# lppllppl920/SAGE-SLAM

Measured on AMD Instinct MI355X. Metric: M residuals/sec (+ LM iters/sec), 64-keyframe feature-metric BA @128x160, higher is better.
Workload: dtype f32; 1 GPU; 64-keyframe window, 128x160x16 feature pyramids (L=4), 32-dim depth code, dense sampling N=16128, 186 links = 372 photometric + 372 geometric directed edges; parallelism=single GPU, collective=none, accepted_steps=988

## Files before the change

include/sage_ba.h:

```cpp
#ifndef SAGE_BA_H_
#define SAGE_BA_H_

#include <stddef.h>
#include <stdint.h>

#ifdef __cplusplus
extern "C" {
#endif

#define SAGE_MAX_LEVELS 8
#define SAGE_POSE_FLOATS 12

#define SAGE_OK 0
#define SAGE_E_INVALID (-1)
#define SAGE_E_UNSUPPORTED (-2)
#define SAGE_E_NOT_PSD (-3)
#define SAGE_E_STATE (-4)
#define SAGE_E_NO_OVERLAP (-5)

typedef struct SageCamera
{
  float fx, fy, cx, cy, w, h;
} SageCamera;

// ... 9 lines not shown

const char *sage_version(void);
const char *sage_error_string(int code);

typedef struct SageWorkspace SageWorkspace;
int sage_workspace_create(void *hip_stream, SageWorkspace **out);
void sage_workspace_destroy(SageWorkspace *ws);


int sage_photometric_jac_error_calculate(
    SageWorkspace *ws, float *AtA_dev, float *Atb_dev, float *error_host, float *num_inliers_host,
    const float *R10_dev, const float *t10_dev, const float *R0_dev, const float *t0_dev,
    const float *R1_dev, const float *t1_dev,
    const float *bias0_dev, const float *basis0_dev, const float *code0_dev, const float *mask1_dev,
    const int64_t *loc1d_dev, const float *homo_dev,
    const float *feat0_dev, const float *feat1_dev, const float *grad1_dev,
    float scale0, const SagePyramid *pyr, float eps, const float *weights_host,
    int N, int FS, int CS);

int sage_photometric_error_calculate(
    SageWorkspace *ws, float *error_host, float *num_inliers_host,
    const float *R10_dev, const float *t10_dev,
    const float *bias0_dev, const float *basis0_dev, const float *code0_dev, const float *mask1_dev,
    const int64_t *loc1d_dev, const float *homo_dev,
    const float *feat0_dev, const float *feat1_dev,
    float scale0, const SagePyramid *pyr, float eps, const float *weights_host,
    int N, int FS, int CS);

int sage_tracker_photo_jac_error_calculate(
    SageWorkspace *ws, int dof, float *AtA_dev, float *Atb_dev, float *error_host, float *num_inliers_host,
    const float *R_dev, const float *t_dev, const float *mask1_dev,
    const float *dpts0_dev, const float *homo_dev, const float *feat0s_dev,
    const float *feat1_dev, const float *grad1_dev,
    const SagePyramid *pyr, float scale0, float eps, const float *weights_dev, int N, int FS);

int sage_tracker_photo_error_calculate(
    SageWorkspace *ws, float *error_host, float *num_inliers_host,
    const float *R_dev, const float *t_dev, const float *mask1_dev,
    const float *dpts0_dev, const float *homo_dev, const float *feat0s_dev, const float *feat1_dev,
    const SagePyramid *pyr, float eps, const float *weights_dev, int N, int FS);

int sage_geometric_jac_error_calculate(
    SageWorkspace *ws, float *AtA_dev, float *Atb_dev, float *error_host, float *num_inliers_host,
    const float *R10_dev, const float *t10_dev, const float *R0_dev, const float *t0_dev,
    const float *R1_dev, const float *t1_dev,
    const float *bias0_dev, const float *basis0_dev, const float *code0_dev,
    const float *dpt1_dev, const float *dpt_grad1_dev, const float *basis1_dev, const float *mask1_dev,
    const int32_t *loc1d_dev, const float *homo_dev,
    float scale0, float scale1, const SageCamera *cam, float eps, float loss_param, float weight,
    int N, int CS);

int sage_geometric_error_calculate(
    SageWorkspace *ws, float *error_host, float *num_inliers_host,
    const float *R10_dev, const float *t10_dev,
    const float *bias0_dev, const float *basis0_dev, const float *code0_dev,
    const float *dpt1_dev, const float *mask1_dev, const int32_t *loc1d_dev, const float *homo_dev,
    float scale0, const SageCamera *cam, float eps, float loss_param, float weight, int N, int CS);

int sage_depth_and_grad(SageWorkspace *ws, float *dpt_dev, float *dpt_grad_dev,
                        const float *bias_dev, const float *basis_dev, const float *code_dev,
                        float scale, int H, int W, int CS);
int sage_gaussian_pyramid_with_grad(SageWorkspace *ws, float *pyr_dev, float *grad_dev,
                                    const float *feat_dev, const float *mask_dev,
                                    const SagePyramid *pyr, int FS);

int sage_bind_thread_to_device(int device);
int sage_solver_helper_cpus(int *cpus, int n);
int sage_solver_placement_moves(void);
int sage_placement_monitor(int enable);
void sage_shutdown(void);
int sage_host_threads_running(void);

void sage_se3_exp(const float *omega, const float *v, float *R, float *t);
void sage_pose_retract(const float *pose, const float *delta6, float *out);
int sage_nearest_psd(const double *M, int n, double *out);
int sage_nearest_psd_reference(const double *M, int n, double *out);
int sage_factor_block_count(int type, int CS);
int sage_factor_hessian_blocks(int type, int CS, const float *AtA_host, const float *Atb_host, int psd_mode,
                               double *G_out, double *g_out, int32_t *dims_out, int32_t *nkeys_out);
int sage_damped_solve_qr_f32(const float *A, const float *b, int n, float damp, float *x);

int sage_block_solve(const double *packed_host, int K, int nlinks, const int32_t *links, int B, double damp,
                     const double *diag_add, const double *g_add, double *delta);
long long sage_solve_lookahead_count(void);

typedef struct SageLmConfig
{
  int max_num_iters;
  float min_grad_thresh;
  float min_param_inc_thresh;
  float init_damp;
  float min_damp, max_damp;
  float damp_dec_factor;
  float damp_inc_factor;
  float jac_update_err_inc_threshold;
  int max_inner_evals;
  float no_overlap_error;
  int linearize_at_candidate;
} SageLmConfig;
void sage_lm_config_default(SageLmConfig *cfg);

typedef int (*SageTrackLinearizeFn)(void *ctx, const float *pose12, float scale, float *AtA, float *Atb, float *error);
typedef int (*SageTrackErrorFn)(void *ctx, const float *pose12, float scale, float *error);

typedef struct SageLmTraceEntry
{
  float damp, error, candidate_error;
  int accepted, relinearized;
} SageLmTraceEntry;

int sage_track_lm(const SageLmConfig *cfg, int dof, SageTrackLinearizeFn lin, SageTrackErrorFn err, void *ctx,
                  float *pose12, float *scale, float *final_error, int *iters,
                  SageLmTraceEntry *trace, int trace_cap, int *trace_len);

typedef struct SageTrackProblem
{
  SageWorkspace *ws;
  int32_t use_photo;
  const float *mask1_dev, *dpts0_dev, *homo_dev, *feat0s_dev, *feat1_dev, *grad1_dev;
  const float *weights_dev;
  SagePyramid pyr;
  float eps;
  int32_t N, FS;
  int32_t use_keypoints, NK;
  const float *kp_dpts0_dev;
  const float *kp_homo0_dev;
  const float *kp_matched_2d_dev;
  const float *kp_matched_dpts1_dev;
  const float *kp_matched_homo1_dev;
  float kp_loss_param;
  float kp_weight;
} SageTrackProblem;
int sage_track_frame(const SageLmConfig *cfg, int dof, const SageTrackProblem *prob,
                     float *pose12, float *scale, float *final_error, int *iters,
                     SageLmTraceEntry *trace, int trace_cap, int *trace_len);

typedef struct SageWindow SageWindow;

typedef struct SageKeyframeView
{
  const float *feat_pyr;
  const float *grad_pyr;
  const float *bias;
  const float *basis;
  const int64_t *loc1d;
  const float *homo;
  int32_t N;
} SageKeyframeView;

typedef struct SageWindowConfig
{
  SagePyramid pyr;
  int32_t FS, CS;
  const float *mask_dev;
  float photo_weights[SAGE_MAX_LEVELS];
  float geo_weight, geo_loss_param, eps;
  float code_prior_weight;
  float scale_prior_weight;
  float pose_prior_weight;
  int32_t use_photo, use_geo;
} SageWindowConfig;

int sage_window_create(const SageWindowConfig *cfg, void *hip_stream, SageWindow **out);
void sage_window_destroy(SageWindow *w);
int sage_window_add_keyframe(SageWindow *w, const SageKeyframeView *view, const float *pose12,
                             const float *code, float scale);
// ... 75 lines not shown
                                        const float *matched_2d, const SageCamera *cam, float eps, float loss_param,
                                        float weight, int N);

enum { SAGE_LOSS_FAIR = 0, SAGE_LOSS_L2 = 1, SAGE_LOSS_HUBER = 2, SAGE_LOSS_UNBIASED = 3 };
int sage_match_geometry_jac_error_calculate(SageWorkspace *ws, float *AtA_dev, float *Atb_dev, float *error_host,
                                            const float *R10, const float *t10, const float *R0, const float *t0,
                                            const float *R1, const float *t1, const float *bias0, const float *bias1,
                                            const float *basis0, const float *basis1, const float *code0,
                                            const float *code1, const float *homo0, const float *matched_homo1,
                                            const int32_t *loc1d_0, const int32_t *matched_loc1d_1, float scale0,
                                            float scale1, float loss_param, float weight, int loss, int N, int CS);
int sage_match_geometry_error_calculate(SageWorkspace *ws, float *error_host, const float *R10, const float *t10,
                                        const float *bias0, const float *bias1, const float *basis0, const float *basis1,
                                        const float *code0, const float *code1, const float *homo0,
                                        const float *matched_homo1, const int32_t *loc1d_0,
                                        const int32_t *matched_loc1d_1, float scale0, float scale1, float loss_param,
                                        float weight, int loss, int N, int CS);
int sage_loop_mg_jac_error_calculate(SageWorkspace *ws, float *AtA_dev, float *Atb_dev, float *error_host,
                                     const float *R10, const float *t10, const float *R0, const float *t0,
                                     const float *R1, const float *t1, const float *unscaled_dpts0,
                                     const float *matched_unscaled_dpts1, const float *homo0, const float *matched_homo1,
                                     float scale0, float scale1, float loss_param, float weight, int N);
int sage_loop_mg_error_calculate(SageWorkspace *ws, float *error_host, const float *R10, const float *t10,
                                 const float *unscaled_dpts0, const float *matched_unscaled_dpts1, const float *homo0,
                                 const float *matched_homo1, float scale0, float scale1, float loss_param, float weight,
                                 int N);
int sage_tracker_match_geom_jac_error_calculate(SageWorkspace *ws, float *AtA_dev, float *Atb_dev, float *error_host,
                                                const float *R, const float *t, const float *sampled_dpts0,
                                                const float *matched_dpts1, const float *homo0,
                                                const float *matched_homo1, float scale0, float loss_param,
                                                float weight, int with_scale, int N);
int sage_tracker_match_geom_error_calculate(SageWorkspace *ws, float *error_host, const float *R, const float *t,
                                            const float *sampled_dpts0, const float *matched_dpts1, const float *homo0,
                                            const float *matched_homo1, float loss_param, float weight, int N);

int sage_cycle_match(SageWorkspace *ws, const float *desc0_dev, const float *desc1_dev, const int64_t *kp_loc1d_0,
                     int K, int C, int H, int W, float cyc_thresh, int64_t *raw_matched_loc1d_1,
                     int64_t *cyc_matched_loc1d_0, int32_t *inlier_flags, int *n_inliers_host);

int sage_sort_locations(SageWorkspace *ws, const int64_t *loc1d_dev, const float *homo_dev, int n, int H, int W,
                        int64_t *loc1d_out_dev, float *homo_out_dev, int *sorted_host);
int sage_valid_locations(SageWorkspace *ws, const float *mask_dev, const SageCamera *cam, int64_t *loc1d_dev,
                         float *homo_dev, int *n_valid_host);
int sage_shuffle_indices(int64_t seed, int64_t n, int64_t *idx_host);
int sage_sample_locations(SageWorkspace *ws, const int64_t *valid_loc1d_dev, const float *valid_homo_dev, int n_valid,
                          int64_t seed, int num_samples, int64_t *loc1d_dev, float *homo_dev, int *n_out_host);

typedef int (*SageAllReduceFn)(double *dev_buf, size_t n, void *user);
int sage_window_set_allreduce(SageWindow *w, SageAllReduceFn fn, void *user);

typedef struct SageShardPlan SageShardPlan;
int sage_shard_plan_create(int K, int nlinks, const int32_t *links, int B, int rank, int world, SageShardPlan **out);
void sage_shard_plan_destroy(SageShardPlan *p);
size_t sage_shard_sep_count(const SageShardPlan *p);
int sage_shard_num_separators(const SageShardPlan *p);
int sage_shard_num_interior(const SageShardPlan *p);
int sage_shard_keyframe_owner(const SageShardPlan *p, int kf);
int sage_shard_keyframe_is_local(const SageShardPlan *p, int kf);
int sage_shard_eliminate(SageShardPlan *p, const double *packed_local_host, double damp, const double *diag_add,
                         const double *g_add, double *sep_out);
int sage_shard_solve(SageShardPlan *p, const double *sep_reduced, double *delta);
int sage_shard_plan_create_domains(int K, int nlinks, const int32_t *links, int B, int domain, int ndomains,
                                   SageShardPlan **out);
int sage_block_solve_domains(const double *packed_host, int K, int nlinks, const int32_t *links, int B, double damp,
                             const double *diag_add, const double *g_add, int ndomains, double *delta);

int sage_window_emulate_peers(SageWindow *w, const double *rest_dev, int n_iterates);
#define SAGE_RCCL_ID_BYTES 128
int sage_rccl_unique_id(unsigned char *id128);
int sage_rccl_comm_create(const unsigned char *id128, int rank, int world, void **comm_out);
void sage_rccl_comm_destroy(void *comm);
int sage_rccl_comm_info(void *comm, int *ranks_out, int *rank_out);
int sage_window_use_rccl(SageWindow *w, void *nccl_comm);

typedef struct SageLmState
{
  double damp, error, candidate_error;
  int accepted, iters;
} SageLmState;
int sage_window_lm_step(SageWindow *w, SageLmState *st, const SageLmConfig *cfg);
int sage_window_lm_run(SageWindow *w, SageLmState *st, const SageLmConfig *cfg, int n, double *trace, int *done);
int sage_window_lm_run_timed(SageWindow *w, SageLmState *st, const SageLmConfig *cfg, int n, double *trace, int *done,
                             double *step_seconds);
int sage_window_sync_variables(SageWindow *w);

#ifdef __cplusplus
}
#endif
#endif
```

sage_slam_amd/build.py:

```python
from __future__ import annotations

import os
import subprocess
import sys
from concurrent.futures import ThreadPoolExecutor

HERE = os.path.dirname(os.path.abspath(__file__))
ROOT = os.path.dirname(HERE)
CSRC = os.path.join(HERE, "csrc")
OBJ = os.path.join(HERE, "csrc", "_obj")
LIB = os.path.join(HERE, "libsage_ba.so")
SOURCES = ["photo_kernels.hip", "geo_kernels.hip", "track_kernels.hip", "producers.hip", "keypoint_kernels.hip", "solve_kernels.hip", "operators.hip", "tracker.hip", "window.hip", "window_build.hip", "window_dist.hip", "window_factors.hip",
           "host_math.cpp", "block_solver.cpp", "host_threads.cpp", "shard_solve.cpp"]
HEADERS = ["sage_device.h", "sage_internal.h", "host_math.h", "block_solver.h", "host_threads.h", "runtime_internal.h", "finalize_bodies.h", "keypoint_batch.h", "window_plan.h", os.path.join(ROOT, "include", "sage_ba.h")]
HIPCC = os.environ.get("HIPCC", "/opt/rocm/bin/hipcc")
HOSTCXX = os.environ.get("HOSTCXX", "/opt/rocm/lib/llvm/bin/clang++")
FLAGS = ["--offload-arch=gfx950", "-O3", "-std=c++17", "-fPIC", "-Wall", "-Wno-unused-function",
         "-I" + os.path.join(ROOT, "include"), "-I" + CSRC]


def kernel_source_sha16() -> str:
    import hashlib
    h = hashlib.sha256()
    for f in ("photo_kernels.hip", "geo_kernels.hip", "sage_device.h", "sage_internal.h"):
        with open(os.path.join(CSRC, f), "rb") as fh:
            h.update(fh.read())
    return h.hexdigest()[:16]


def _mtime(p):
    return os.path.getmtime(p) if os.path.exists(p) else 0.0


def _compile(src):
    obj = os.path.join(OBJ, os.path.splitext(src)[0] + ".o")
    deps = [os.path.join(CSRC, src)] + [h if os.path.isabs(h) else os.path.join(CSRC, h) for h in HEADERS]
    if _mtime(obj) >= max(_mtime(d) for d in deps):
        return obj, False
    if src.endswith(".hip"):
        cmd = [HIPCC] + FLAGS + ["-x", "hip", "-c", os.path.join(CSRC, src), "-o", obj]
    else:
        cmd = [HOSTCXX, "-O3", "-std=c++17", "-fPIC", "-Wall", "-I" + os.path.join(ROOT, "include"), "-I" + CSRC,
               "-c", os.path.join(CSRC, src), "-o", obj]
    subprocess.check_call(cmd)
    return obj, True


def build(force: bool = False, verbose: bool = False) -> str:
    os.makedirs(OBJ, exist_ok=True)
    if force:
        for f in os.listdir(OBJ):
            os.remove(os.path.join(OBJ, f))
    with ThreadPoolExecutor(max_workers=min(8, len(SOURCES))) as ex:
        res = list(ex.map(_compile, SOURCES))
    objs = [o for o, _ in res]
    if any(ch for _, ch in res) or not os.path.exists(LIB):
        subprocess.check_call([HIPCC, "--offload-arch=gfx950", "-shared", "-fPIC", "-o", LIB] + objs + ["-lpthread"])
        if verbose:
            print("built", LIB)
    return LIB


GLUE_SRC = os.path.join(ROOT, "integration", "compile_check", "prepass_run.cpp")
GLUE_BIN = os.path.join(ROOT, "integration", "compile_check", "_bin", "prepass_run")
REF_THIRDPARTY = "/root/reference/system/thirdparty"


def build_glue_check(verbose: bool = False):
    if not os.path.isdir(REF_THIRDPARTY):
        return GLUE_BIN if os.path.exists(GLUE_BIN) else None
    deps = [GLUE_SRC, os.path.join(ROOT, "integration", "sage_gtsam_prepass.h"), os.path.join(ROOT, "include", "sage_ba.h"),
            os.path.join(ROOT, "integration", "compile_check", "gtsam", "linear", "HessianFactor.h"),
            os.path.join(ROOT, "integration", "compile_check", "gtsam", "nonlinear", "Values.h"), LIB]
    if _mtime(GLUE_BIN) >= max(_mtime(d) for d in deps):
        return GLUE_BIN
    os.makedirs(os.path.dirname(GLUE_BIN), exist_ok=True)
    subprocess.check_call([HOSTCXX, "-std=c++17", "-O1", "-w", "-D__HIP_PLATFORM_AMD__", "-I" + os.path.join(ROOT, "include"),
                           "-I" + os.path.join(ROOT, "integration", "compile_check"), "-I" + REF_THIRDPARTY + "/eigen",
                           "-I" + REF_THIRDPARTY + "/Sophus", "-I/opt/rocm/include", GLUE_SRC, "-o", GLUE_BIN,
                           "-L" + HERE, "-lsage_ba", "-L/opt/rocm/lib", "-lamdhip64",
                           "-Wl,-rpath,$ORIGIN/../../../sage_slam_amd", "-Wl,-rpath,/opt/rocm/lib"])
    if verbose:
        print("built", GLUE_BIN)
    return GLUE_BIN


ADAPTER_BIN = os.path.join(ROOT, "integration", "compile_check", "_bin", "adapter_run")
REF_SYSTEM = "/root/reference/system"


def build_adapter_run(verbose: bool = False):
    if not os.path.isdir(REF_SYSTEM):
        return ADAPTER_BIN if os.path.exists(ADAPTER_BIN) else None
    import torch
    T = os.path.dirname(torch.__file__)
    srcs = [os.path.join(ROOT, "integration", "sage_adapter.cpp"), os.path.join(ROOT, "integration", "sage_adapter_keypoints.cpp"),
            os.path.join(ROOT, "integration", "compile_check", "adapter_run.cpp")]
# ... 31 lines not shown
```

sage_slam_amd/capi.py:

```python
from __future__ import annotations

import ctypes as C
import os
from typing import List, Optional, Sequence

import numpy as np

HERE = os.path.dirname(os.path.abspath(__file__))
LIB_PATH = os.path.join(HERE, "libsage_ba.so")
SAGE_MAX_LEVELS = 8


class SageError(RuntimeError):
    def __init__(self, code: int, where: str):
        self.code = code
        msg = lib().sage_error_string(code).decode() if _lib is not None else "?"
        super().__init__(f"{where}: {msg} (code {code})")


class SageCamera(C.Structure):
    _fields_ = [(n, C.c_float) for n in ("fx", "fy", "cx", "cy", "w", "h")]


class SagePyramid(C.Structure):
    _fields_ = [("levels", C.c_int32), ("P", C.c_int32), ("level_offsets", C.c_int32 * SAGE_MAX_LEVELS),
                ("cam", SageCamera * SAGE_MAX_LEVELS)]


class SageLmConfig(C.Structure):
    _fields_ = [("max_num_iters", C.c_int), ("min_grad_thresh", C.c_float), ("min_param_inc_thresh", C.c_float),
                ("init_damp", C.c_float), ("min_damp", C.c_float), ("max_damp", C.c_float),
                ("damp_dec_factor", C.c_float), ("damp_inc_factor", C.c_float),
                ("jac_update_err_inc_threshold", C.c_float), ("max_inner_evals", C.c_int),
                ("no_overlap_error", C.c_float), ("linearize_at_candidate", C.c_int)]


class SageLmTraceEntry(C.Structure):
    _fields_ = [("damp", C.c_float), ("error", C.c_float), ("candidate_error", C.c_float),
                ("accepted", C.c_int), ("relinearized", C.c_int)]


class SageTrackProblem(C.Structure):
    _fields_ = [("ws", C.c_void_p), ("use_photo", C.c_int32), ("mask1_dev", C.c_void_p), ("dpts0_dev", C.c_void_p),
                ("homo_dev", C.c_void_p), ("feat0s_dev", C.c_void_p), ("feat1_dev", C.c_void_p),
                ("grad1_dev", C.c_void_p), ("weights_dev", C.c_void_p), ("pyr", SagePyramid), ("eps", C.c_float),
                ("N", C.c_int32), ("FS", C.c_int32), ("use_keypoints", C.c_int32), ("NK", C.c_int32),
                ("kp_dpts0_dev", C.c_void_p), ("kp_homo0_dev", C.c_void_p), ("kp_matched_2d_dev", C.c_void_p),
                ("kp_matched_dpts1_dev", C.c_void_p), ("kp_matched_homo1_dev", C.c_void_p),
                ("kp_loss_param", C.c_float), ("kp_weight", C.c_float)]


class SageKeyframeView(C.Structure):
    _fields_ = [("feat_pyr", C.c_void_p), ("grad_pyr", C.c_void_p), ("bias", C.c_void_p), ("basis", C.c_void_p),
                ("loc1d", C.c_void_p), ("homo", C.c_void_p), ("N", C.c_int32)]


class SageWindowConfig(C.Structure):
    _fields_ = [("pyr", SagePyramid), ("FS", C.c_int32), ("CS", C.c_int32), ("mask_dev", C.c_void_p),
                ("photo_weights", C.c_float * SAGE_MAX_LEVELS), ("geo_weight", C.c_float),
                ("geo_loss_param", C.c_float), ("eps", C.c_float), ("code_prior_weight", C.c_float),
                ("scale_prior_weight", C.c_float), ("pose_prior_weight", C.c_float),
                ("use_photo", C.c_int32), ("use_geo", C.c_int32)]


SAGE_KP_REPROJECTION, SAGE_KP_MATCH_GEOMETRY = 0, 1


class SageKeypointTerm(C.Structure):
    _fields_ = [("kind", C.c_int32), ("edge", C.c_int32), ("N", C.c_int32), ("loc1d_0", C.c_void_p), ("homo0", C.c_void_p),
                ("matched_2d", C.c_void_p), ("matched_loc1d_1", C.c_void_p), ("matched_homo1", C.c_void_p),
                ("loss_param", C.c_float), ("weight", C.c_float), ("loss", C.c_int32)]


ALLREDUCE_FN = C.CFUNCTYPE(C.c_int, C.c_void_p, C.c_size_t, C.c_void_p)


class SageLmState(C.Structure):
    _fields_ = [("damp", C.c_double), ("error", C.c_double), ("candidate_error", C.c_double),
                ("accepted", C.c_int), ("iters", C.c_int)]


TRACK_LIN_FN = C.CFUNCTYPE(C.c_int, C.c_void_p, C.POINTER(C.c_float), C.c_float, C.POINTER(C.c_float),
                           C.POINTER(C.c_float), C.POINTER(C.c_float))
TRACK_ERR_FN = C.CFUNCTYPE(C.c_int, C.c_void_p, C.POINTER(C.c_float), C.c_float, C.POINTER(C.c_float))

_lib = None

SYMBOLS = [
    "sage_camera_pyramid", "sage_version", "sage_error_string", "sage_workspace_create", "sage_workspace_destroy",
    "sage_photometric_jac_error_calculate", "sage_photometric_error_calculate",
    "sage_tracker_photo_jac_error_calculate", "sage_tracker_photo_error_calculate",
    "sage_geometric_jac_error_calculate", "sage_geometric_error_calculate", "sage_depth_and_grad",
    "sage_gaussian_pyramid_with_grad", "sage_se3_exp", "sage_pose_retract", "sage_nearest_psd", "sage_nearest_psd_reference", "sage_factor_block_count", "sage_factor_hessian_blocks",
    "sage_damped_solve_qr_f32", "sage_block_solve", "sage_solve_lookahead_count", "sage_lm_config_default", "sage_track_lm", "sage_track_frame",
    "sage_window_create", "sage_window_destroy", "sage_window_add_keyframe", "sage_window_add_link", "sage_window_set_link_geo_loss",
    "sage_window_set_shard", "sage_window_finalize", "sage_window_num_keyframes", "sage_window_num_links",
    "sage_window_block_size", "sage_window_packed_count", "sage_window_packed_dev",
    "sage_window_residuals_per_linearize", "sage_window_bytes_per_linearize", "sage_window_linearize",
    "sage_window_error", "sage_window_tune_runs", "sage_window_set_runs", "sage_window_error_dev", "sage_window_solve", "sage_window_total_error",
    "sage_window_accept", "sage_window_reset", "sage_window_get_keyframe", "sage_window_set_keyframe", "sage_window_get_delta",
    "sage_window_get_edge", "sage_window_add_keypoint_term", "sage_window_num_keypoint_terms", "sage_window_get_keypoint_term", "sage_window_prepass", "sage_window_factor", "sage_window_factor_error", "sage_window_prepare_factors", "sage_factor_psd", "sage_factor_cut_blocks", "sage_window_set_profiling", "sage_window_get_kernel_time", "sage_window_get_phase_time", "sage_window_lm_step", "sage_window_lm_run", "sage_window_lm_run_timed", "sage_window_sync_variables", "sage_window_set_allreduce", "sage_shard_plan_create", "sage_shard_plan_create_domains", "sage_block_solve_domains", "sage_shard_plan_destroy", "sage_shard_sep_count", "sage_shard_num_separators", "sage_shard_num_interior", "sage_shard_keyframe_owner", "sage_shard_keyframe_is_local", "sage_shard_eliminate", "sage_shard_solve", "sage_rccl_unique_id", "sage_rccl_comm_create", "sage_rccl_comm_destroy", "sage_rccl_comm_info", "sage_window_use_rccl", "sage_window_emulate_peers", "sage_sort_locations", "sage_bind_thread_to_device", "sage_solver_helper_cpus", "sage_solver_placement_moves", "sage_placement_monitor", "sage_shutdown", "sage_host_threads_running",
    "sage_valid_locations", "sage_shuffle_indices", "sage_sample_locations",
    "sage_reprojection_jac_error_calculate", "sage_reprojection_error_calculate",
    "sage_tracker_reproj_jac_error_calculate", "sage_tracker_reproj_error_calculate",
    "sage_match_geometry_jac_error_calculate", "sage_match_geometry_error_calculate",
    "sage_loop_mg_jac_error_calculate", "sage_loop_mg_error_calculate",
    "sage_tracker_match_geom_jac_error_calculate", "sage_tracker_match_geom_error_calculate", "sage_cycle_match",
]


def lib():
    global _lib
    if _lib is None:
        LIB_PATH = os.environ.get("SAGE_BA_LIB", globals()["LIB_PATH"])
        if not os.path.exists(LIB_PATH):
            raise ImportError(f"{LIB_PATH} is missing: run `python -m sage_slam_amd.build` "
                              "(the HIP engine has no fallback path)")
        import torch
        L = C.CDLL(LIB_PATH)
        L.sage_version.restype = C.c_char_p
        L.sage_error_string.restype = C.c_char_p
        L.sage_window_packed_count.restype = C.c_size_t
        L.sage_shutdown.restype = None
        L.sage_window_packed_dev.restype = C.c_void_p
        L.sage_window_error_dev.restype = C.c_void_p
        L.sage_window_residuals_per_linearize.restype = C.c_double
        L.sage_window_bytes_per_linearize.restype = C.c_double
        for name in ("sage_window_packed_count", "sage_window_packed_dev", "sage_window_error_dev",
                     "sage_window_residuals_per_linearize", "sage_window_bytes_per_linearize",
                     "sage_window_num_keyframes", "sage_window_num_links", "sage_window_block_size"):
            getattr(L, name).argtypes = [C.c_void_p]
        _lib = L
    return _lib


def _chk(code: int, where: str):
    if code != 0:
        raise SageError(code, where)


def _f32(a) -> np.ndarray:
    return np.ascontiguousarray(a, dtype=np.float32)


def _fp(a: np.ndarray):
    return a.ctypes.data_as(C.POINTER(C.c_float))


def dptr(t) -> C.c_void_p:
    if t is None:
        return C.c_void_p(0)
    assert t.is_contiguous(), "device buffers handed to the C ABI must be contiguous"
    return C.c_void_p(t.data_ptr())


def make_pyramid(cam, levels: int) -> SagePyramid:
    base = SageCamera(*[float(v) for v in (cam.fx, cam.fy, cam.cx, cam.cy, cam.w, cam.h)])
    out = SagePyramid()
    _chk(lib().sage_camera_pyramid(C.byref(base), levels, C.byref(out)), "sage_camera_pyramid")
    return out


def se3_exp(omega, v):
    omega = _f32(omega); v = _f32(v)
    R = np.zeros(9, np.float32); t = np.zeros(3, np.float32)
    lib().sage_se3_exp(_fp(omega), _fp(v), _fp(R), _fp(t))
    return R.reshape(3, 3), t


def pose_retract(pose12, delta6):
    pose12 = _f32(pose12).reshape(12); delta6 = _f32(delta6)
    out = np.zeros(12, np.float32)
    lib().sage_pose_retract(_fp(pose12), _fp(delta6), _fp(out))
    return out


def nearest_psd(M):
    M = np.ascontiguousarray(M, dtype=np.float64)
    out = np.zeros_like(M)
    _chk(lib().sage_nearest_psd(M.ctypes.data_as(C.POINTER(C.c_double)), M.shape[0],
                                out.ctypes.data_as(C.POINTER(C.c_double))), "sage_nearest_psd")
    return out


def nearest_psd_reference(M):
    M = np.ascontiguousarray(M, np.float64)
    out = np.zeros_like(M)
    _chk(lib().sage_nearest_psd_reference(M.ctypes.data_as(C.POINTER(C.c_double)), M.shape[0],
                                          out.ctypes.data_as(C.POINTER(C.c_double))), "sage_nearest_psd_reference")
    return out


def factor_hessian_blocks(type_: int, CS: int, AtA, Atb, psd_mode: int = 1):
    L = lib()
    A = _f32(AtA); b = _f32(Atb)
    n = L.sage_factor_block_count(type_, CS)
    if n < 0:
        raise SageError(n, "sage_factor_block_count")
    G = np.zeros(n, np.float64); g = np.zeros(b.size, np.float64)
    dims = (C.c_int32 * 6)(); nk = C.c_int32()
    _chk(L.sage_factor_hessian_blocks(type_, CS, _fp(A), _fp(b), psd_mode, G.ctypes.data_as(C.POINTER(C.c_double)),
                                      g.ctypes.data_as(C.POINTER(C.c_double)), dims, C.byref(nk)),
         "sage_factor_hessian_blocks")
    dims = [int(dims[i]) for i in range(nk.value)]
    blocks, o = {}, 0
    for i in range(nk.value):
        for j in range(i, nk.value):
            blocks[(i, j)] = G[o:o + dims[i] * dims[j]].reshape(dims[i], dims[j]); o += dims[i] * dims[j]
    offs = np.concatenate([[0], np.cumsum(dims)])
    return blocks, [g[offs[i]:offs[i + 1]] for i in range(nk.value)], dims


def damped_solve_qr_f32(A, b, damp):
    A = _f32(A); b = _f32(b)
    x = np.zeros(b.shape[0], np.float32)
    _chk(lib().sage_damped_solve_qr_f32(_fp(A), _fp(b), b.shape[0], C.c_float(damp), _fp(x)), "sage_damped_solve_qr_f32")
    return x


def block_solve(packed, K, links, B, damp, diag_add=None, g_add=None):
    packed = np.ascontiguousarray(packed, dtype=np.float64)
    lk = np.ascontiguousarray(np.asarray(links, dtype=np.int32).reshape(-1))
    delta = np.zeros(K * B, np.float64)
    dp = lambda a: None if a is None else np.ascontiguousarray(a, np.float64).ctypes.data_as(C.POINTER(C.c_double))
    da = None if diag_add is None else np.ascontiguousarray(diag_add, np.float64)
    ga = None if g_add is None else np.ascontiguousarray(g_add, np.float64)
    _chk(lib().sage_block_solve(packed.ctypes.data_as(C.POINTER(C.c_double)), K, len(lk) // 2, lk.ctypes.data_as(C.POINTER(C.c_int32)), B,
                                C.c_double(damp), dp(da), dp(ga), delta.ctypes.data_as(C.POINTER(C.c_double))),
         "sage_block_solve")
    return delta


def solve_lookahead_count() -> int:
    f = lib().sage_solve_lookahead_count
    f.restype = C.c_longlong
    return int(f())


def block_solve_domains(packed, K, links, B, damp, ndomains, diag_add=None, g_add=None):
    p = np.ascontiguousarray(packed, np.float64)
    lk = np.ascontiguousarray(np.asarray(links, np.int32).reshape(-1))
    out = np.zeros(K * B, np.float64)
    dp = lambda a: None if a is None else np.ascontiguousarray(a, np.float64).ctypes.data_as(C.POINTER(C.c_double))
    da = None if diag_add is None else np.ascontiguousarray(diag_add, np.float64)
    ga = None if g_add is None else np.ascontiguousarray(g_add, np.float64)
    _chk(lib().sage_block_solve_domains(p.ctypes.data_as(C.POINTER(C.c_double)), K, len(links),
                                        lk.ctypes.data_as(C.POINTER(C.c_int32)), B, C.c_double(damp), dp(da), dp(ga),
                                        ndomains, out.ctypes.data_as(C.POINTER(C.c_double))), "sage_block_solve_domains")
    return out


def lm_config_default() -> SageLmConfig:
    cfg = SageLmConfig()
    lib().sage_lm_config_default(C.byref(cfg))
    return cfg


def pack_pose(R, t) -> np.ndarray:
    return np.concatenate([_f32(R).reshape(9), _f32(t).reshape(3)])


def track_lm(cfg: SageLmConfig, dof: int, lin_fn, err_fn, pose12, scale: float, trace_cap: int = 256):
    def _lin(ctx, p, s, AtA, Atb, err):
        A, b, e = lin_fn(np.ctypeslib.as_array(p, (12,)).copy(), float(s))
        A = _f32(A).reshape(-1); b = _f32(b).reshape(-1)
        for i in range(dof * dof):
            AtA[i] = A[i]
        for i in range(dof):
            Atb[i] = b[i]
        err[0] = e
        return 0

    def _err(ctx, p, s, err):
        err[0] = err_fn(np.ctypeslib.as_array(p, (12,)).copy(), float(s))
        return 0

    pose = _f32(pose12).reshape(12).copy()
    sc = C.c_float(scale)
    fe = C.c_float(0); it = C.c_int(0); tl = C.c_int(0)
    trace = (SageLmTraceEntry * trace_cap)()
    cb1, cb2 = TRACK_LIN_FN(_lin), TRACK_ERR_FN(_err)
    _chk(lib().sage_track_lm(C.byref(cfg), dof, cb1, cb2, None, _fp(pose), C.byref(sc), C.byref(fe), C.byref(it),
                             trace, trace_cap, C.byref(tl)), "sage_track_lm")
    tr = [dict(damp=trace[i].damp, error=trace[i].error, candidate_error=trace[i].candidate_error,
               accepted=trace[i].accepted, relinearized=trace[i].relinearized) for i in range(tl.value)]
    return pose, sc.value, fe.value, it.value, tr


def track_frame(cfg: SageLmConfig, dof: int, prob: "SageTrackProblem", pose12, scale: float, trace_cap: int = 256):
    L = lib()
    p = _f32(pose12).copy()
    sc = C.c_float(scale); fe = C.c_float(); it = C.c_int(); tl = C.c_int()
    tr = (SageLmTraceEntry * trace_cap)()
    rc = L.sage_track_frame(C.byref(cfg), dof, C.byref(prob), _fp(p), C.byref(sc), C.byref(fe), C.byref(it), tr,
                            trace_cap, C.byref(tl))
    trace = [dict(damp=tr[i].damp, error=tr[i].error, candidate_error=tr[i].candidate_error,
                  accepted=tr[i].accepted, relinearized=tr[i].relinearized) for i in range(tl.value)]
    return rc, p, sc.value, fe.value, it.value, trace


class Workspace:

    def __init__(self, stream=None):
        self.h = C.c_void_p()
        sp = C.c_void_p(stream.cuda_stream) if stream is not None else C.c_void_p(0)
        _chk(lib().sage_workspace_create(sp, C.byref(self.h)), "sage_workspace_create")

    def close(self):
        if self.h:
            lib().sage_workspace_destroy(self.h)
            self.h = C.c_void_p()

    def __del__(self):
# ... 257 lines not shown
    def tune_runs(self):
        tpb, rule = C.c_int(0), C.c_int(0)
        ms_rule, ms_best = C.c_float(0), C.c_float(0)
        _chk(lib().sage_window_tune_runs(self.h, C.byref(tpb), C.byref(rule), C.byref(ms_rule), C.byref(ms_best)),
             "sage_window_tune_runs")
        return dict(tpb=tpb.value, tpb_rule=rule.value, ms_rule=ms_rule.value, ms_best=ms_best.value)

    def set_runs(self, tpb):
        _chk(lib().sage_window_set_runs(self.h, int(tpb)), "sage_window_set_runs")

    def solve(self, damp, want_norm=True):
        if not want_norm:
            _chk(lib().sage_window_solve(self.h, C.c_double(damp), None), "sage_window_solve")
            return None
        sn = C.c_double()
        _chk(lib().sage_window_solve(self.h, C.c_double(damp), C.byref(sn)), "sage_window_solve")
        return sn.value

    def total_error(self, from_linearize: bool):
        e = C.c_double()
        _chk(lib().sage_window_total_error(self.h, int(from_linearize), C.byref(e)), "sage_window_total_error")
        return e.value

    def accept(self):
        _chk(lib().sage_window_accept(self.h), "sage_window_accept")

    def reset(self):
        _chk(lib().sage_window_reset(self.h), "sage_window_reset")

    def set_allreduce(self, dist_module, group=None):
        tensors = {}
        for t in (self.packed_tensor(), self.error_tensor()):
            tensors[(t.data_ptr(), t.numel())] = t

        def hook(ptr, n, _user):
            try:
                t = tensors.get((ptr, n))
                if t is None:
                    t = tensors[(ptr, n)] = _tensor_from_ptr(ptr, n)
                dist_module.all_reduce(t, group=group)
                return 0
            except Exception:
                import traceback
                traceback.print_exc()
                return 1

        self._allreduce_cb = ALLREDUCE_FN(hook)
        _chk(lib().sage_window_set_allreduce(self.h, self._allreduce_cb, None), "sage_window_set_allreduce")

    def sync_variables(self):
        _chk(lib().sage_window_sync_variables(self.h), "sage_window_sync_variables")

    def use_rccl(self, comm):
        _chk(lib().sage_window_use_rccl(self.h, C.c_void_p(comm)), "sage_window_use_rccl")

    def emulate_peers(self, rest):
        if rest is None:
            self._emu_rest = None
            _chk(lib().sage_window_emulate_peers(self.h, None, 0), "sage_window_emulate_peers")
            return
        assert rest.is_cuda and rest.dim() == 2 and rest.shape[1] == self.packed_count and rest.is_contiguous()
        self._emu_rest = rest
        _chk(lib().sage_window_emulate_peers(self.h, C.c_void_p(rest.data_ptr()), int(rest.shape[0])),
             "sage_window_emulate_peers")

    def lm_step(self, state: SageLmState, cfg: SageLmConfig):
        _chk(lib().sage_window_lm_step(self.h, C.byref(state), C.byref(cfg)), "sage_window_lm_step")
        return state

    def lm_run(self, state: SageLmState, cfg: SageLmConfig, n: int):
        tr = np.zeros((n, 4), np.float64)
        done = C.c_int()
        _chk(lib().sage_window_lm_run(self.h, C.byref(state), C.byref(cfg), n, tr.ctypes.data_as(C.POINTER(C.c_double)),
                                      C.byref(done)), "sage_window_lm_run")
        return tr[:done.value]

    def lm_run_timed(self, state: SageLmState, cfg: SageLmConfig, n: int):
        tr = np.zeros((n, 4), np.float64); sec = np.zeros(n, np.float64)
        done = C.c_int()
        _chk(lib().sage_window_lm_run_timed(self.h, C.byref(state), C.byref(cfg), n, tr.ctypes.data_as(C.POINTER(C.c_double)),
                                            C.byref(done), sec.ctypes.data_as(C.POINTER(C.c_double))), "sage_window_lm_run_timed")
        return tr[:done.value], sec[:done.value]

    def delta(self):
        d = np.zeros(self.K * self.B, np.float64)
        _chk(lib().sage_window_get_delta(self.h, d.ctypes.data_as(C.POINTER(C.c_double))), "sage_window_get_delta")
        return d

    def get_keyframe(self, k):
        pose = np.zeros(12, np.float32); code = np.zeros(self.win.CS, np.float32); s = C.c_float()
        _chk(lib().sage_window_get_keyframe(self.h, k, _fp(pose), _fp(code), C.byref(s)), "sage_window_get_keyframe")
        return pose, code, s.value

    def set_keyframe(self, k, pose12, code, scale):
        pose12 = _f32(pose12); code = _f32(code)
        _chk(lib().sage_window_set_keyframe(self.h, k, _fp(pose12), _fp(code), C.c_float(scale)),
             "sage_window_set_keyframe")

    def get_edge(self, type_, e):
        D = 13 + self.win.CS if type_ == 0 else 14 + 2 * self.win.CS
        A = np.zeros((D, D), np.float32); b = np.zeros(D, np.float32)
        err = C.c_float(); nin = C.c_float()
        _chk(lib().sage_window_get_edge(self.h, type_, e, _fp(A), _fp(b), C.byref(err), C.byref(nin)),
             "sage_window_get_edge")
        return dict(AtA=A, Atb=b, error=err.value, num_inliers=nin.value)

    def prepass(self, poses12, codes, scales, jacobians: bool = True) -> bool:
        P = _f32(np.asarray(poses12).reshape(-1)); Cd = _f32(np.asarray(codes).reshape(-1)); S = _f32(np.asarray(scales).reshape(-1))
        K = self.K
        assert P.size == K * 12 and Cd.size == K * self.win.CS and S.size == K
        rec = C.c_int32()
        _chk(lib().sage_window_prepass(self.h, _fp(P), _fp(Cd), _fp(S), int(jacobians), C.byref(rec)), "sage_window_prepass")
        return bool(rec.value)

    def factor(self, type_, e, psd_mode: int = 1):
        L = lib(); CS = self.win.CS
        n = L.sage_factor_block_count(type_, CS)
        D = 13 + CS if type_ == 0 else 14 + 2 * CS
        G = np.zeros(n, np.float64); g = np.zeros(D, np.float64); f = C.c_double()
        dims = (C.c_int32 * 6)(); nk = C.c_int32()
        _chk(L.sage_window_factor(self.h, type_, e, psd_mode, G.ctypes.data_as(C.POINTER(C.c_double)),
                                  g.ctypes.data_as(C.POINTER(C.c_double)), C.byref(f), dims, C.byref(nk)), "sage_window_factor")
        dims = [int(dims[i]) for i in range(nk.value)]
        blocks, o = {}, 0
        for i in range(nk.value):
            for j in range(i, nk.value):
                blocks[(i, j)] = G[o:o + dims[i] * dims[j]].reshape(dims[i], dims[j]); o += dims[i] * dims[j]
        offs = np.concatenate([[0], np.cumsum(dims)])
        return blocks, [g[offs[i]:offs[i + 1]] for i in range(nk.value)], f.value, dims

    def prepare_factors(self, psd_mode: int = 1, n_threads: int = 0):
        _chk(lib().sage_window_prepare_factors(self.h, psd_mode, n_threads), "sage_window_prepare_factors")

    def factor_error(self, type_, e) -> float:
        v = C.c_double()
        _chk(lib().sage_window_factor_error(self.h, type_, e, C.byref(v)), "sage_window_factor_error")
        return v.value

    def set_profiling(self, on):
        _chk(lib().sage_window_set_profiling(self.h, int(on)), "sage_window_set_profiling")

    def kernel_time(self, which: int):
        ms = C.c_double(); n = C.c_int()
        _chk(lib().sage_window_get_kernel_time(self.h, which, C.byref(ms), C.byref(n)), "sage_window_get_kernel_time")
        return ms.value, n.value

    def phase_time(self):
        ms = (C.c_double * 4)(); n = C.c_int()
        _chk(lib().sage_window_get_phase_time(self.h, ms, C.byref(n)), "sage_window_get_phase_time")
        return dict(zip(("linearize", "allreduce", "solve", "error_pass"), (float(v) for v in ms))), n.value

    def packed_host(self):
        return self.packed_tensor().cpu().numpy()

    def close(self):
        if self.h:
            lib().sage_window_destroy(self.h)
            self.h = C.c_void_p()

    def __del__(self):
        try:
            self.close()
        except Exception:
            pass


# ... 350 lines not shown
```

sage_slam_amd/csrc/block_solver.cpp:

```cpp
#include <algorithm>
#include <atomic>
#include <chrono>
#include <cmath>
#include <cstdio>
#include <cstdlib>
#include <cstring>
#include <sched.h>
#include <thread>
#include <vector>

#include "block_solver.h"
#include "host_math.h"
#include "sage_ba.h"

namespace sage
{
namespace
{
typedef double v8d __attribute__((vector_size(64), aligned(8)));

#define SAGE_LOADU(dst, p) __builtin_memcpy(&(dst), (p), sizeof(v8d))
#define SAGE_STOREU(p, v) __builtin_memcpy((p), &(v), sizeof(v8d))

struct RowPrefetch
// ... 1492 lines not shown
  {
    const int rc = block_chol_range(E0, T, X, y, 0, K);
    return rc ? rc : block_back_range(E0, T, X, y, 0, K);
  }
  const int sep0 = E0.n1 + E0.n2;
  BlockEnvelope E = E0;
  const bool arrow = block_plan_has_arrow_rows(E0);
  SepJob job;
  SepPool *pool = nullptr;
  if (arrow)
  {
    job.E = &E; job.T = T; job.X = X; job.y = y;
    sep_job_build(job);
    job.t_start = mono_seconds();
    E.progress = job.progress;
    pool = pool_engage(job);
  }
  BlockEnvelope::RowPipe pipes[2];
  E.pipe = pipes;
  static const bool no_sep_pre = sage::env_flag("SAGE_SOLVE_NO_SEP_PRE");
  E.sep_pre = !arrow && !no_sep_pre;
  CholHelper *h = helper_engage(E, T, X, y);
  const bool piped = lookahead_engage(1, E, T, X, y, 0, E.n1);
  const bool dbg = debug_timing();
  double tp[6] = {0, 0, 0, 0, 0, 0};
  auto lap = [&](int k) {
    if (dbg)
      tp[k] = mono_seconds();
  };
  lap(0);
  int rc = block_chol_range(E, T, X, y, 0, E.n1, piped ? RowRole::chain : RowRole::whole);
  if (piped)
    lookahead_release(1);
  lap(1);
  const bool helper_has_it = h && helper_claimed(h);
  const int rc2 = helper_has_it ? helper_join_factor(h) : rc == 0 ? block_chol_range(E, T, X, y, E.n1, sep0) : 0;
  lap(2);
  if (rc == 0)
    rc = rc2;
  if (arrow)
    rc = arrow_separator(job, rc, tp[2]);
  else if (rc == 0)
    rc = block_chol_range(E, T, X, y, sep0, K);
  if (rc == 0)
    block_back_range(E, T, X, y, sep0, K);
  if (arrow)
  {
    arrow_back_substitute(job, E, rc);
    if (pool)
      pool_release(pool);
  }
  lap(3);
  if (helper_has_it)
    helper_go_back(h, rc == 0);
  if (rc == 0)
  {
    block_back_range(E, T, X, y, 0, E.n1);
    if (!helper_has_it)
      block_back_range(E, T, X, y, E.n1, sep0);
  }
  lap(4);
  if (helper_has_it)
    helper_join_back(h);
  lap(5);
  if (dbg)
    fprintf(stderr, "[sage block chol] us: first half %.0f (+wait for the %s %.0f) separator %.0f%s back-subst %.0f (+wait %.0f)\n",
            1e6 * (tp[1] - tp[0]), helper_has_it ? "helper" : "second half, same thread", 1e6 * (tp[2] - tp[1]),
            1e6 * (tp[3] - tp[2]), arrow ? (pool ? " (arrow rows, worker pool)" : " (arrow rows, no pool)") : "",
            1e6 * (tp[4] - tp[3]), 1e6 * (tp[5] - tp[4]));
  if (h)
    helper_release(h);
  return rc;
}

BlockEnvelope envelope_of(const BlockPlan &plan, int Bp)
{
  BlockEnvelope env;
  env.K = (int)plan.row_first.size(); env.Bp = Bp; env.n1 = plan.n1; env.n2 = plan.n2;
  env.row_first = plan.row_first.data(); env.row_off = plan.row_off.data();
  env.a_first = plan.a_first.data(); env.a_cnt = plan.a_cnt.data(); env.a_off = plan.a_off.data();
  env.col_ptr = plan.col_ptr.data(); env.col_rows = plan.col_rows.data();
  return env;
}
}

extern "C" long long sage_solve_lookahead_count(void) { return sage::g_lookahead_count.load(); }

extern "C" int sage_block_solve(const double *packed, int K, int nlinks, const int32_t *links, int B, double damp,
                                const double *diag_add, const double *g_add, double *delta)
{
  if (!packed || K < 1 || B < 1 || nlinks < 0 || (nlinks > 0 && !links) || !delta)
    return SAGE_E_INVALID;
  const int Bp = sage::padded_block(B);
  if (Bp == 0)
    return SAGE_E_UNSUPPORTED;
  const int BB = B * B, BBp = Bp * Bp;
  const double *diag = packed;
  const double *lnk = diag + (size_t)K * BB;
  const double *g = lnk + (size_t)nlinks * BB;
  std::vector<std::pair<int, int>> lk(nlinks);
  for (int l = 0; l < nlinks; ++l)
    lk[l] = {links[2 * l], links[2 * l + 1]};
  sage::BlockPlan bp;
  int rcp = sage::plan_blocks(K, lk, !sage::env_flag("SAGE_SOLVE_NO_SPLIT"), bp);
  if (rcp == SAGE_E_UNSUPPORTED)
  {
    std::sort(lk.begin(), lk.end());
    lk.erase(std::unique(lk.begin(), lk.end()), lk.end());
    rcp = sage::plan_blocks(K, lk, !sage::env_flag("SAGE_SOLVE_NO_SPLIT"), bp);
  }
  if (rcp != SAGE_OK)
    return rcp;
  const int nblk = bp.nblk;
  std::vector<double> T((size_t)nblk * BBp, 0.0), X((size_t)K * BBp), y((size_t)K * Bp, 0.0);
  for (int q = 0; q < K; ++q)
  {
    const int k = bp.perm[q];
    double *D = T.data() + (size_t)bp.index(q, q) * BBp;
    for (int i = 0; i < Bp; ++i)
      for (int j = 0; j < Bp; ++j)
      {
        double v = 0.0;
        if (i < B && j < B)
        {
          v = 0.5 * (diag[(size_t)k * BB + i * B + j] + diag[(size_t)k * BB + j * B + i]);
          if (i == j)
            v = (v + (diag_add ? diag_add[k * B + i] : 0.0)) * (1.0 + damp);
        }
        else if (i == j)
          v = 1.0 + damp;
        D[i * Bp + j] = v;
      }
    for (int i = 0; i < B; ++i)
      y[(size_t)q * Bp + i] = g[(size_t)k * B + i] + (g_add ? g_add[k * B + i] : 0.0);
  }
  for (int l = 0; l < nlinks; ++l)
  {
    const int a = links[2 * l], b = links[2 * l + 1];
    const int qi = std::max(bp.pos[a], bp.pos[b]), qj = std::min(bp.pos[a], bp.pos[b]);
    double *D = T.data() + (size_t)bp.index(qi, qj) * BBp;
    const bool row_is_a = bp.perm[qi] == a;
    for (int i = 0; i < B; ++i)
      for (int j = 0; j < B; ++j)
        D[row_is_a ? j * Bp + i : i * Bp + j] += lnk[(size_t)l * BB + i * B + j];
  }
  static const bool dbg = sage::env_flag("SAGE_DEBUG_TIMING");
  const auto t0 = std::chrono::steady_clock::now();
  sage::BlockEnvelope env = sage::envelope_of(bp, Bp);
  int rcf;
  {
    sage::SolveLease lease;
    if (bp.n1 > 0)
      env.no_lookahead = sage::block_chol_arm(sage::block_plan_has_arrow_rows(env), sage::block_plan_long_arrow_chains(env));
    rcf = sage::block_chol_solve_tr(env, T.data(), X.data(), y.data());
  }
  if (dbg)
    fprintf(stderr, "[sage block_solve] fixed-block Cholesky + substitution %.3f ms\n",
            std::chrono::duration<double, std::milli>(std::chrono::steady_clock::now() - t0).count());
  if (rcf != 0)
    return SAGE_E_NOT_PSD;
  for (int k = 0; k < K; ++k)
    std::memcpy(delta + (size_t)k * B, y.data() + (size_t)bp.pos[k] * Bp, sizeof(double) * B);
  return SAGE_OK;
}
```

sage_slam_amd/csrc/block_solver.h:

```cpp
#pragma once
#include <stdint.h>

#include <algorithm>
#include <atomic>
#include <utility>
#include <vector>

#include "host_threads.h"

namespace sage
{
inline int padded_block(int B) { return B < 1 ? 0 : B <= 24 ? 24 : B <= 40 ? 40 : 0; }

struct BlockEnvelope
{
  int K = 0, Bp = 0;
  const int32_t *row_first = nullptr, *row_off = nullptr;
  const int32_t *a_first = nullptr, *a_cnt = nullptr, *a_off = nullptr;
  int n1 = 0, n2 = 0;
  const volatile unsigned *ready = nullptr;
  unsigned epoch = 0;
  const uint8_t *fill = nullptr;
  bool no_lookahead = false;
  std::atomic<int> *progress = nullptr;
  const int32_t *col_ptr = nullptr, *col_rows = nullptr;
  int bs_skip_from = 0x7fffffff;
  struct RowPipe
  {
    alignas(64) std::atomic<int> early{0};
    alignas(64) std::atomic<int> late{0};
    alignas(64) std::atomic<int> pre{0};
  };
  RowPipe *pipe = nullptr;
  bool sep_pre = false;

  struct Range
  {
    int lo, hi;
  };
  Range a_range(int i) const
  {
    const int a = a_cnt ? a_first[i] : 0;
    return {a, a + (a_cnt ? a_cnt[i] : 0)};
  }
  Range b_range(int i) const { return {row_first[i], i}; }
  bool has(int i, int j) const
  {
    const Range a = a_range(i);
    return (j >= row_first[i] && j <= i) || (j >= a.lo && j < a.hi);
  }
  size_t index(int i, int j) const
  {
    return (size_t)(j < row_first[i] ? a_off[i] + j - a_first[i] : row_off[i] + j - row_first[i]);
  }
  double *block(double *T, int i, int j) const { return T + index(i, j) * (size_t)(Bp * Bp); }
  Range sep_range(int srow, int half) const
  {
    if (half == 0)
      return a_range(srow);
    const int sep0 = n1 + n2;
    return {std::min((int)row_first[srow], sep0), sep0};
  }
};
int block_chol_solve_tr(const BlockEnvelope &env, double *T, double *X, double *y);
int block_chol_partial(const BlockEnvelope &env, double *T, double *X, double *y, int nI);
int block_chol_partial_back(const BlockEnvelope &env, double *T, double *X, double *y, int nI);
int block_plan_long_arrow_chains(const BlockEnvelope &env);
bool block_plan_has_arrow_rows(const BlockEnvelope &env);

struct BlockPlan
{
  std::vector<int32_t> perm, pos, row_first, row_off, a_first, a_cnt, a_off, blk_row, blk_col, blk_src;
  std::vector<int32_t> col_ptr, col_rows;
  int nblk = 0, n1 = 0, n2 = 0;
  int index(int i, int j) const
  {
    return j < row_first[i] ? a_off[i] + j - a_first[i] : row_off[i] + j - row_first[i];
  }
};
int plan_blocks(int K, const std::vector<std::pair<int, int>> &links, bool allow_split, BlockPlan &out);
BlockEnvelope envelope_of(const BlockPlan &plan, int Bp);
}
```

sage_slam_amd/csrc/runtime_internal.h:

```cpp
#pragma once

#include <hip/hip_runtime.h>

#include <algorithm>
#include <atomic>
#include <cctype>
#include <sched.h>
#include <chrono>
#include <cmath>
#include <cstdlib>
#include <cstdio>
#include <cstring>
#include <thread>
#include <vector>

#include <dlfcn.h>
#if __has_include(<rccl/rccl.h>)
#include <rccl/rccl.h>
#else
extern "C"
{
  typedef struct ncclComm *ncclComm_t;
  typedef struct
  {
    char internal[128];
  } ncclUniqueId;
  typedef enum { ncclSuccess = 0 } ncclResult_t;
  typedef enum { ncclSum = 0 } ncclRedOp_t;
  typedef enum { ncclDouble = 8 } ncclDataType_t;
}
#endif

#include "host_math.h"
#include "host_threads.h"
#include "sage_ba.h"
#include "sage_internal.h"
#include "keypoint_batch.h"

using namespace sage;

#define SAGE_HIP(expr)                \
  do                                  \
  {                                   \
    hipError_t _e = (expr);           \
    if (_e != hipSuccess)             \
      return (int)_e;                 \
  } while (0)

namespace sage_rt
{

struct DevBuf
{
  void *p = nullptr;
  size_t cap = 0;
  int reserve(size_t bytes)
  {
    if (bytes <= cap)
      return 0;
    if (p)
      (void)hipFree(p);
    p = nullptr;
    cap = 0;
    hipError_t e = hipMalloc(&p, bytes);
    if (e != hipSuccess)
      return (int)e;
    cap = bytes;
    return 0;
  }
  void release()
  {
    if (p)
      (void)hipFree(p);
    p = nullptr;
    cap = 0;
  }
  template <class T>
  T *as() const { return reinterpret_cast<T *>(p); }
};

inline int pick_tiles_per_block(long long total_tiles)
{
  if (total_tiles >= 8192)
    return 4;
  if (total_tiles >= 4096)
    return 2;
  return 1;
}

struct WorkList
{
  std::vector<WorkItem> work;
  std::vector<int32_t> edge_first, edge_tiles;
  std::vector<int32_t> rec_first, rec_count;
  int tiles_per_block = 1;
  int flush = 1;
  int n_records = 0;
  void build(const std::vector<int> &N, int tpb_override = 0, const std::vector<int> *order = nullptr, int flush_ = 0)
  {
    long long total = 0;
    for (int n : N)
      total += (n + kTile - 1) / kTile;
    tiles_per_block = tpb_override > 0 ? tpb_override : pick_tiles_per_block(total);
    flush = (flush_ > 0 && flush_ < tiles_per_block && tiles_per_block % flush_ == 0) ? flush_ : tiles_per_block;
    work.clear();
    edge_first.assign(N.size(), 0);
    edge_tiles.assign(N.size(), 0);
    rec_first.assign(N.size(), 0);
    rec_count.assign(N.size(), 0);
    n_records = 0;
    for (size_t i = 0; i < N.size(); ++i)
    {
      const size_t e = order ? (size_t)(*order)[i] : i;
      const int tiles = (N[e] + kTile - 1) / kTile;
      edge_first[e] = (int32_t)work.size();
      for (int t = 0; t < tiles; t += tiles_per_block)
        work.push_back(WorkItem{(int32_t)e, t});
      edge_tiles[e] = (int32_t)work.size() - edge_first[e];
      rec_first[e] = n_records;
      rec_count[e] = (tiles + flush - 1) / flush;
      n_records += rec_count[e];
    }
  }
};

}
using namespace sage_rt;

struct SageWorkspace
{
  hipStream_t stream = nullptr;
  DevBuf work, edge_first, edge_tiles, partials, misc, dpt0;
  float *host_stats = nullptr;
  unsigned ticket_epoch = 0;
  int cached_N = -1;
  int n_work = 0;
  int tiles_per_block = 1;
  bool defer_fetch = false;
  float *stats_ptr = nullptr;
  DevBuf trk_dpts, trk_kp_dpts;
  float *trk_host = nullptr;
};

static inline float *ws_stats(SageWorkspace *ws) { return ws->stats_ptr ? ws->stats_ptr : ws->host_stats; }
int ws_ticket_wait(SageWorkspace *ws);


static inline bool supported(int CS, int FS)
{
  return (CS == 16 || CS == 32) && (FS == 16 || FS == 32);
}

namespace sage
{
struct AdjEntry
{
  int32_t type;
  int32_t edge;
  int32_t role;
};

struct LinkEdges
{
  int32_t e_ab, e_ba;
};

struct AssembleParams
{
  const float *AtA_p, *Atb_p, *stats_p;
  const float *AtA_g, *Atb_g, *stats_g;
  const double *wide_p, *wide_g;
  const int32_t *adj_start;
  const AdjEntry *adj;
  const LinkEdges *links;
  double *packed;
  double *tail_mirror;
  int K, nlinks, CS, n_edges_p, n_edges_g;
  int split;
  const int32_t *blocks;
  const float *AtA_kr, *Atb_kr, *AtA_km, *Atb_km, *stats_k;
  const int32_t *link_kp_start;
  const AdjEntry *link_kp;
  int n_kr, n_km;
};

struct KpTotals
{
  const float *stats;
  int n_kr, n_km;
};

struct ErrorTotalsSide
{
  const int32_t *edge_first, *edge_tiles;
  const float *partials;
  float *stats;
  float fallback, scale;
  int n_edges;
  int stride, err_off, cnt_off;
};

}

struct SageWindow
{
  SageWindowConfig cfg;
  hipStream_t stream = nullptr;
  bool finalized = false;
  int rank = 0, world = 1;
  int K = 0, B = 0, VS = 0;
  std::vector<SageKeyframeView> views;
  std::vector<float> pose[2], code[2], scale[2];
  std::vector<float> link_geo_loss;
  std::vector<float> code_init, scale_init, pose_init;
  std::vector<float> code_added;
  std::vector<std::pair<int, int>> links;
  std::vector<int> local_links;
  std::vector<int> local_edges;
  int n_edges = 0;
  DevBuf vars[2];
  DevBuf wide_p, wide_g;
  DevBuf sorted_loc, sorted_homo;
  std::vector<std::pair<const int64_t *, const float *>> user_samples;
  std::vector<int> user_n;
  DevBuf dpt, dgrad, depth_items[2];
  int n_depth = 0;
  int dpt_set = -1;
  bool dgrad_valid = false;
  SageAllReduceFn allreduce = nullptr;
  void *allreduce_user = nullptr;
  void *rccl_hook = nullptr;
  SageShardPlan *shard = nullptr;
  DevBuf sepbuf;
  std::vector<double> h_sep;
  double *h_err = nullptr;
  uint64_t mirror_epoch = 0;
  const double *emu_rest = nullptr;
  int emu_n = 0, emu_cur = 0;
  uint64_t err_epoch = 0;
  DevBuf geo_px;
  bool merge_ok = false;
  DevBuf pk;
  DevBuf f0s;
  DevBuf ptab[2], gtab[2];
  DevBuf work_p, first_p, tiles_p, work_g, first_g, tiles_g;
  DevBuf rec_first_p, rec_count_p;
  int flush_p = 0, n_rec_p = 0;
  std::vector<int> Nedge;
  int tpb_heur = 1;
  DevBuf part_p, part_g;
  DevBuf AtA_p, Atb_p, stats_p, AtA_g, Atb_g, stats_g;
  DevBuf adj_start, adj, link_edges, packed, errbuf;
  int n_work_p = 0, n_work_g = 0, tpb_p = 1, tpb_g = 1;
  std::vector<double> host_packed;
  std::vector<double> delta;
  sage::DeviceSolver *solver = nullptr;
  bool cand_pending = false;
  double residuals_per_lin = 0, bytes_per_lin = 0;
  bool have_lin = false;
  uint64_t vars_epoch = 1, lin_epoch = 0;
  bool spec_err_valid = false;
  bool packed_reduced = false;
  double spec_error = 0.0;
  DevBuf packed_save;
  DevBuf packed_loc;
  DevBuf asm_blocks;
  int n_asm_blocks = 0;
  struct KeypointTermHost
  {
    int32_t kind, edge, N, loss;
    float loss_param, weight;
    std::vector<int32_t> loc0, loc1;
    std::vector<float> homo0, second;
  };
  std::vector<KeypointTermHost> kp_added;
  std::vector<int> kp_local;
  int n_kr = 0, n_km = 0;
  bool kp_lin = false;
  DevBuf kp_pool, kp_table, kp_link_start, kp_link;
  DevBuf AtA_kr, Atb_kr, AtA_km, Atb_km, stats_k;
  int (*allreduce2)(const double *send, double *recv, size_t n, void *user) = nullptr;
  struct FactorCache
  {
    bool lin = false, err = false;
    std::vector<float> pose, code, scale;
    std::vector<float> Ap, bp, sp, Ag, bg, sg;
    std::vector<double> Cp, Cg;
    int psd_mode = -1;
  } fc;
  struct PhaseMarks
  {
    std::vector<std::pair<int, hipEvent_t>> ev;
  };
  std::vector<PhaseMarks> phase_pending;
  PhaseMarks phase_cur;
  double phase_ms[4] = {0, 0, 0, 0};
  int phase_n = 0;
  bool profiling = false;
  int prof_level = 0;
  std::vector<std::pair<hipEvent_t, hipEvent_t>> pending[6];
  std::vector<hipEvent_t> ev_free;
  double prof_ms[6] = {0, 0, 0, 0, 0, 0};
  int prof_n[6] = {0, 0, 0, 0, 0, 0};
};


template <class T>
static int upload(DevBuf &b, const std::vector<T> &v, hipStream_t s)
{
  int rc = b.reserve(std::max<size_t>(v.size(), 1) * sizeof(T));
  if (rc)
    return rc;
  if (!v.empty())
    SAGE_HIP(hipMemcpyAsync(b.p, v.data(), v.size() * sizeof(T), hipMemcpyHostToDevice, s));
  return 0;
}
int window_upload_vars(SageWindow *w, int set);
int window_local_edge(const SageWindow *w, int global_edge);
int window_linearize_set(SageWindow *w, int set, double *dst = nullptr, bool local_blocks = false, bool merge = false);
int window_sync_candidate(SageWindow *w, bool stream_idle = false);
void window_phase_mark(SageWindow *w, int which);
```

sage_slam_amd/csrc/solve_kernels.hip:

```cpp
#include <algorithm>
#include <cmath>
#include <cstdio>
#include <chrono>
#include <cstdlib>
#include <cstring>
#include <vector>

#include "block_solver.h"
#include "host_math.h"
#include "sage_device.h"
#include "sage_internal.h"

namespace sage
{

struct SolvePlan
{
  int K, B, Bp, nblk, nlinks;
  const int32_t *row_first;
  const int32_t *row_off;
  const int32_t *blk_row, *blk_col, *blk_src;
  const int32_t *perm, *pos;
};

struct SolvePriors
{
  double code_w, scale_w, pose_w;
  float scale_init0;
  float pose_init0[12];
};

__device__ inline void pose_local_dev(const float *origin, const float *other, double out[6])
{
  double Rr[9];
  for (int i = 0; i < 3; ++i)
    for (int j = 0; j < 3; ++j)
      Rr[i * 3 + j] = (double)other[i * 3 + 0] * origin[j * 3 + 0] + (double)other[i * 3 + 1] * origin[j * 3 + 1] +
                      (double)other[i * 3 + 2] * origin[j * 3 + 2];
  for (int i = 0; i < 3; ++i)
    out[i] = other[9 + i] - (Rr[i * 3 + 0] * origin[9] + Rr[i * 3 + 1] * origin[10] + Rr[i * 3 + 2] * origin[11]);
  const double tr = Rr[0] + Rr[4] + Rr[8];
  const double cs = fmin(1.0, fmax(-1.0, 0.5 * (tr - 1.0)));
  const double th = acos(cs);
  const double k = th < 1e-8 ? 0.5 : th / (2.0 * sin(th));
  out[3] = k * (Rr[7] - Rr[5]);
  out[4] = k * (Rr[2] - Rr[6]);
  out[5] = k * (Rr[3] - Rr[1]);
}

__global__ __launch_bounds__(256) void solve_scatter_kernel(const SolvePlan P, const double *__restrict__ packed,
                                                            const float *__restrict__ vars0, int VS, int CS,
                                                            const SolvePriors pri, double damp, int transposed,
                                                            double *__restrict__ L, double *__restrict__ y,
                                                            const int32_t *__restrict__ order, unsigned *flags,
                                                            unsigned epoch, int first, int count, int deliver_fill)
{
  const int tid = threadIdx.x;
  const int B = P.B, Bp = P.Bp, BB = B * B;
  __shared__ double s_dadd[64], s_gadd[64];
  for (int it = first + blockIdx.x; it < first + count; it += gridDim.x)
  {
    const int b = order ? order[it] : it;
    const int i = P.blk_row[b], j = P.blk_col[b], srcf = P.blk_src[b];
    const int src = srcf < 0 ? -1 : (srcf & 0x3fffffff);
    const bool flip = srcf >= 0 && (srcf & 0x40000000);
    if (flags && src < 0 && i != j && !deliver_fill)
      continue;
    const int kf = P.perm[i];
    const double *diag = packed + (size_t)kf * BB;
    const double *lnk = packed + (size_t)P.K * BB + (size_t)(src < 0 ? 0 : src) * BB;
    const double *g = packed + (size_t)P.K * BB + (size_t)P.nlinks * BB + (size_t)kf * B;
    double *out = L + (size_t)b * Bp * Bp;
    if (i == j)
    {
      const float *var = vars0 + (size_t)kf * VS;
      if (tid < B)
      {
        double da = 0.0, ga = 0.0;
        if (tid >= 6 && tid < 6 + CS)
        {
          da = pri.code_w;
          ga = pri.code_w * (0.0 - (double)var[13 + tid - 6]);
        }
        if (kf == 0 && tid == 6 + CS && pri.scale_w > 0)
        {
          const double s = (double)var[12];
          da = pri.scale_w / (s * s);
          ga = pri.scale_w / s * (log((double)pri.scale_init0) - log(s));
        }
        if (kf == 0 && tid < 6 && pri.pose_w > 0)
        {
          double loc[6];
          pose_local_dev(var, pri.pose_init0, loc);
          da = pri.pose_w;
          ga = pri.pose_w * loc[tid];
        }
        s_dadd[tid] = da;
        s_gadd[tid] = ga;
      }
      __syncthreads();
    }
    for (int o = tid; o < Bp * Bp; o += blockDim.x)
    {
      const int hi = o / Bp, lo = o - hi * Bp;
      const int r = transposed ? lo : hi, c = transposed ? hi : lo;
      double v = 0.0;
      if (i == j)
      {
        if (r < B && c < B)
        {
          v = 0.5 * (diag[r * B + c] + diag[c * B + r]);
          if (r == c)
            v = (v + s_dadd[r]) * (1.0 + damp);
        }
        else if (r == c)
          v = 1.0 + damp;
      }
      else if (src >= 0 && r < B && c < B)
        v = flip ? lnk[r * B + c] : lnk[c * B + r];
      out[o] = v;
    }
    if (i == j)
      for (int r = tid; r < Bp; r += blockDim.x)
        y[(size_t)i * Bp + r] = r < B ? g[r] + s_gadd[r] : 0.0;
    if (flags)
    {
      __syncthreads();
      if (tid == 0)
      {
        __threadfence_system();
        *reinterpret_cast<volatile unsigned *>(flags + b) = epoch;
      }
    }
    else
      __syncthreads();
  }
}

__device__ inline void se3_exp_dev(const float *omega, const float *v, float *R, float *t)
{
  float theta = sqrtf(omega[0] * omega[0] + omega[1] * omega[1] + omega[2] * omega[2]);
  float n[3] = {1.f, 0.f, 0.f};
  if (theta > 0)
  {
    n[0] = omega[0] / theta;
    n[1] = omega[1] / theta;
    n[2] = omega[2] / theta;
  }
  theta = fmaxf(theta, 1.0e-14f);
  const float s = sinf(theta), c = cosf(theta);
  const float Km[3][3] = {{0, -n[2], n[1]}, {n[2], 0, -n[0]}, {-n[1], n[0], 0}};
  float K2[3][3];
  for (int i = 0; i < 3; ++i)
    for (int j = 0; j < 3; ++j)
      K2[i][j] = Km[i][0] * Km[0][j] + Km[i][1] * Km[1][j] + Km[i][2] * Km[2][j];
  const float a = (1.0f - c) / theta, b = (theta - s) / theta;
  for (int i = 0; i < 3; ++i)
  {
    float acc = 0.f;
    for (int j = 0; j < 3; ++j)
    {
      const float id = (i == j) ? 1.f : 0.f;
      R[i * 3 + j] = id + s * Km[i][j] + (1.0f - c) * K2[i][j];
      acc += (id + a * Km[i][j] + b * K2[i][j]) * v[j];
    }
    t[i] = acc;
  }
}

__global__ __launch_bounds__(1024) void solve_retract_kernel(const double *__restrict__ x, int K, int B, int Bp, int CS,
                                                            int VS, const int32_t *__restrict__ pos,
                                                            const float *__restrict__ vars0,
                                                            float *__restrict__ vars1, float *__restrict__ h_vars,
                                                            double *__restrict__ h_delta, double *__restrict__ h_tail,
                                                            const volatile unsigned *go, unsigned epoch)
{
  const int tid = threadIdx.x;
  __shared__ int s_go;
  if (tid == 0)
  {
    const unsigned long long t0 = wall_clock64();
    unsigned v;
    bool timed_out = false;
    for (;;)
    {
      v = *go;
      const unsigned d = ((v & 0x7fffffffu) - epoch) & 0x7fffffffu;
      if (d == 0u)
        break;
      if (d < 0x40000000u && (v & 0x7fffffffu) != 0u)
      {
        v = 0x80000000u;
        break;
      }
      __builtin_amdgcn_s_sleep(4);
      if (wall_clock64() - t0 > 200000000ull)
      {
        v = 0x80000000u;
        timed_out = true;
        break;
      }
    }
    __threadfence_system();
    s_go = (v & 0x80000000u) ? 0 : 1;
    *reinterpret_cast<volatile int *>(h_tail + 1) = timed_out ? 2 : (s_go ? 0 : 1);
  }
  __syncthreads();
  if (!s_go)
    return;
  double nrm = 0.0;
  for (int idx = tid; idx < K * B; idx += blockDim.x)
  {
    const int k = idx / B, r = idx - k * B;
    const double d = x[(size_t)pos[k] * Bp + r];
    h_delta[idx] = d;
    nrm += d * d;
    const float *v0 = vars0 + (size_t)k * VS;
    if (r >= 6)
    {
      const int slot = r < 6 + CS ? 13 + r - 6 : 12;
      const float v = v0[slot] + (float)d;
      vars1[(size_t)k * VS + slot] = v;
      h_vars[(size_t)k * VS + slot] = v;
    }
  }
  for (int k = tid; k < K; k += blockDim.x)
  {
    const double *xk = x + (size_t)pos[k] * Bp;
    const float *v0 = vars0 + (size_t)k * VS;
    float d6[6], dR[9], dt[3], o[12];
    for (int i = 0; i < 6; ++i)
      d6[i] = (float)xk[i];
    se3_exp_dev(d6 + 3, d6, dR, dt);
    for (int i = 0; i < 3; ++i)
    {
      for (int j = 0; j < 3; ++j)
        o[i * 3 + j] = dR[i * 3 + 0] * v0[0 * 3 + j] + dR[i * 3 + 1] * v0[1 * 3 + j] + dR[i * 3 + 2] * v0[2 * 3 + j];
      o[9 + i] = dR[i * 3 + 0] * v0[9] + dR[i * 3 + 1] * v0[10] + dR[i * 3 + 2] * v0[11] + dt[i];
    }
    for (int i = 0; i < 12; ++i)
    {
      vars1[(size_t)k * VS + i] = o[i];
      h_vars[(size_t)k * VS + i] = o[i];
    }
  }
  __shared__ double s_n[16];
  for (int off = 32; off > 0; off >>= 1)
    nrm += __shfl_down(nrm, off);
  if ((tid & 63) == 0)
    s_n[tid >> 6] = nrm;
  __syncthreads();
  if (tid == 0)
  {
    double tot = 0.0;
    for (int w = 0; w < (int)(blockDim.x >> 6); ++w)
      tot += s_n[w];
    h_tail[0] = tot;
  }
}

struct DeviceSolver
{
  int K = 0, B = 0, Bp = 0, nblk = 0, nlinks = 0;
  void *d_int = nullptr;
  void *h_pinned = nullptr;
  size_t h_go_off = 0;
  unsigned go_epoch = 0;
  size_t h_vars_off = 0, h_delta_off = 0, h_tail_off = 0, h_bytes = 0;
  SolvePlan plan{};
  int VS = 0;
  void *h_T = nullptr, *h_y = nullptr;
  std::vector<double> h_X;
  BlockPlan host_plan;
  const int32_t *d_order = nullptr;
  unsigned *h_flags = nullptr;
  unsigned epoch = 0;
  int scatter_wgs = 32;
  std::vector<uint8_t> h_fill;
};

int solver_create(DeviceSolver **out, int K, int B, int VS, const std::vector<std::pair<int, int>> &links,
                  hipStream_t stream, bool allow_split)
{
  *out = nullptr;
  const int Bp = sage::padded_block(B);
  if (Bp == 0 || K < 1)
    return SAGE_E_UNSUPPORTED;
  BlockPlan bp;
  {
    const int rcp = plan_blocks(K, links, allow_split && !sage::env_flag("SAGE_SOLVE_NO_SPLIT"), bp);
    if (rcp != SAGE_OK)
      return rcp;
  }
  const int n1 = bp.n1, n2 = bp.n2, nblk = bp.nblk;
  const std::vector<int32_t> &perm = bp.perm, &pos = bp.pos, &row_first = bp.row_first, &row_off = bp.row_off,
                             &a_cnt = bp.a_cnt, &a_off = bp.a_off, &blk_row = bp.blk_row, &blk_col = bp.blk_col,
                             &blk_src = bp.blk_src;
  DeviceSolver *S = new DeviceSolver;
  S->K = K; S->B = B; S->Bp = Bp; S->nblk = nblk; S->nlinks = (int)links.size(); S->VS = VS;
  std::vector<int32_t> all;
  auto put = [&](const std::vector<int32_t> &v) {
    const size_t off = all.size();
    all.insert(all.end(), v.begin(), v.end());
    while (all.size() % 4)
      all.push_back(0);
    return off;
  };
  const size_t o_rf = put(row_first), o_ro = put(row_off), o_br = put(blk_row), o_bc = put(blk_col),
               o_bs = put(blk_src), o_pm = put(perm), o_ps = put(pos);
  std::vector<int32_t> order;
  {
    auto push_row = [&](int i) {
      for (int q = 0; q < a_cnt[i]; ++q)
        order.push_back(a_off[i] + q);
      for (int q = 0; q <= i - row_first[i]; ++q)
        order.push_back(row_off[i] + q);
    };
    if (n1 > 0)
    {
      for (int t = 0; t < std::max(n1, n2); ++t)
      {
        if (t < n1)
          push_row(t);
        if (t < n2)
          push_row(n1 + t);
      }
      for (int i = n1 + n2; i < K; ++i)
        push_row(i);
    }
    else
      for (int i = 0; i < K; ++i)
        push_row(i);
  }
  const size_t o_ord = put(order);
  auto fail = [&](int rc) {
    solver_destroy(S);
    return rc;
  };
  if (hipMalloc(&S->d_int, all.size() * sizeof(int32_t)) != hipSuccess)
    return fail((int)hipErrorOutOfMemory);
  if (hipMemcpyAsync(S->d_int, all.data(), all.size() * sizeof(int32_t), hipMemcpyHostToDevice, stream) != hipSuccess)
    return fail((int)hipErrorUnknown);
  if (hipStreamSynchronize(stream) != hipSuccess)
    return fail((int)hipErrorUnknown);
  const size_t ty_doubles = (size_t)nblk * Bp * Bp + (size_t)K * Bp;
  {
    if (hipHostMalloc(&S->h_T, ty_doubles * sizeof(double) + (size_t)nblk * sizeof(unsigned), hipHostMallocDefault) !=
        hipSuccess)
      return fail((int)hipErrorOutOfMemory);
    S->h_y = reinterpret_cast<double *>(S->h_T) + (size_t)nblk * Bp * Bp;
    S->h_flags = reinterpret_cast<unsigned *>(reinterpret_cast<double *>(S->h_T) + ty_doubles);
    std::memset(S->h_flags, 0, (size_t)nblk * sizeof(unsigned));
    S->h_X.assign((size_t)K * Bp * Bp, 0.0);
  }
  S->h_vars_off = 0;
  S->h_delta_off = ((size_t)K * VS * sizeof(float) + 15) / 16 * 16;
  S->h_tail_off = S->h_delta_off + (size_t)K * B * sizeof(double);
  S->h_go_off = S->h_tail_off + 2 * sizeof(double);
  S->h_bytes = S->h_go_off + 2 * sizeof(double);
  if (hipHostMalloc(&S->h_pinned, S->h_bytes, hipHostMallocDefault) != hipSuccess)
    return fail((int)hipErrorOutOfMemory);
  const int32_t *base = reinterpret_cast<const int32_t *>(S->d_int);
  SolvePlan &P = S->plan;
  P.K = K; P.B = B; P.Bp = Bp; P.nblk = nblk; P.nlinks = (int)links.size();
  P.row_first = base + o_rf; P.row_off = base + o_ro;
  P.blk_row = base + o_br; P.blk_col = base + o_bc; P.blk_src = base + o_bs; P.perm = base + o_pm; P.pos = base + o_ps;
  S->d_order = base + o_ord;
  S->h_fill.assign((size_t)nblk, 0);
  for (int b = 0; b < nblk; ++b)
    S->h_fill[b] = (blk_src[b] < 0 && blk_row[b] != blk_col[b]) ? 1 : 0;
  if (const char *e = getenv("SAGE_SCATTER_WGS"))
    S->scatter_wgs = std::max(1, atoi(e));
  std::memset(S->h_pinned, 0, S->h_bytes);
  S->host_plan = std::move(bp);
  *out = S;
  return SAGE_OK;
}

void solver_destroy(DeviceSolver *S)
{
  if (!S)
    return;
  void *bufs[] = {S->d_int};
  for (void *p : bufs)
    if (p)
      (void)hipFree(p);
  void *hbufs[] = {S->h_pinned, S->h_T};
  for (void *p : hbufs)
    if (p)
      (void)hipHostFree(p);
  delete S;
}

int solver_run(DeviceSolver *S, hipStream_t stream, const double *packed_dev, const float *vars0, float *vars1,
               int CS, double damp, double code_w, double scale_w, double pose_w, float scale_init0,
               const float *pose_init0)
{
  SolvePriors pri{};
  pri.code_w = code_w; pri.scale_w = scale_w; pri.pose_w = pose_w; pri.scale_init0 = scale_init0;
  for (int i = 0; i < 12; ++i)
    pri.pose_init0[i] = pose_init0[i];
  {
    static const bool dbgt = sage::env_flag("SAGE_DEBUG_TIMING");
    hipError_t eh;
    SolveLease lease;
    BlockEnvelope env = envelope_of(S->host_plan, S->Bp);
    if (env.n1 > 0)
      env.no_lookahead = block_chol_arm(block_plan_has_arrow_rows(env), block_plan_long_arrow_chains(env));
    S->epoch += 1;
    if (S->epoch == 0)
      S->epoch = 1;
    hipLaunchKernelGGL(solve_scatter_kernel, dim3(std::min(S->scatter_wgs, S->nblk)), dim3(256), 0, stream, S->plan,
                       packed_dev, vars0, S->VS, CS, pri, damp, 1, reinterpret_cast<double *>(S->h_T),
                       reinterpret_cast<double *>(S->h_y), S->d_order, S->h_flags, S->epoch, 0, S->nblk,
                       sage::env_flag("SAGE_SCATTER_FILL") ? 1 : 0);
    if ((eh = hipGetLastError()) != hipSuccess)
      return (int)eh;
    char *hp = reinterpret_cast<char *>(S->h_pinned);
    volatile unsigned *go = reinterpret_cast<volatile unsigned *>(hp + S->h_go_off);
    S->go_epoch = (S->go_epoch + 1) & 0x7fffffffu;
    if (S->go_epoch == 0)
      S->go_epoch = 1;
    hipLaunchKernelGGL(solve_retract_kernel, dim3(1), dim3(1024), 0, stream,
                       reinterpret_cast<const double *>(S->h_y), S->K, S->B, S->Bp, CS, S->VS, S->plan.pos, vars0, vars1,
                       reinterpret_cast<float *>(hp + S->h_vars_off), reinterpret_cast<double *>(hp + S->h_delta_off),
                       reinterpret_cast<double *>(hp + S->h_tail_off), go, S->go_epoch);
    if ((eh = hipGetLastError()) != hipSuccess)
      return (int)eh;
    struct GoGuard
    {
      volatile unsigned *go;
      unsigned word;
      ~GoGuard()
      {
        std::atomic_thread_fence(std::memory_order_release);
        *go = word;
      }
    } guard{go, S->go_epoch | 0x80000000u};
    const auto t1 = std::chrono::steady_clock::now();
    env.ready = S->h_flags; env.epoch = S->epoch;
    env.fill = S->h_fill.data();
    const int bad = block_chol_solve_tr(env, reinterpret_cast<double *>(S->h_T), S->h_X.data(),
                                        reinterpret_cast<double *>(S->h_y));
    const auto t2 = std::chrono::steady_clock::now();
    if (dbgt)
      fprintf(stderr, "[sage hybrid solve] wait for the system + host cholesky %.3f ms\n",
              std::chrono::duration<double, std::milli>(t2 - t1).count());
    if (bad == -2)
      return SAGE_E_STATE;
    if (bad)
      return SAGE_E_NOT_PSD;
    guard.word = S->go_epoch;
    (void)eh;
  }
  return SAGE_OK;
}

const float *solver_host_vars(const DeviceSolver *S) { return reinterpret_cast<const float *>(reinterpret_cast<const char *>(S->h_pinned) + S->h_vars_off); }
const double *solver_host_delta(const DeviceSolver *S) { return reinterpret_cast<const double *>(reinterpret_cast<const char *>(S->h_pinned) + S->h_delta_off); }
double solver_host_step_norm2(const DeviceSolver *S) { return *reinterpret_cast<const double *>(reinterpret_cast<const char *>(S->h_pinned) + S->h_tail_off); }
int solver_host_status(const DeviceSolver *S) { return *reinterpret_cast<const int *>(reinterpret_cast<const char *>(S->h_pinned) + S->h_tail_off + sizeof(double)); }

}
```

sage_slam_amd/csrc/window.hip:

```cpp
#include "runtime_internal.h"
#include "finalize_bodies.h"

namespace sage
{




__device__ __forceinline__ int edge_col(int type, int role, int bi, int CS)
{
  if (bi < 6)
    return role * 6 + bi;
  if (type == 0)
  {
    if (role == 1)
      return -1;
    return bi < 6 + CS ? 12 + (bi - 6) : 12 + CS;
  }
  if (bi < 6 + CS)
    return 12 + role * CS + (bi - 6);
  return 12 + 2 * CS + role;
}

template <bool KP>
__global__ __launch_bounds__(1024) void assemble_kernel(const AssembleParams p)
{
  const int B = 7 + p.CS, BB = B * B;
  const int Dp = 13 + p.CS, Dg = 14 + 2 * p.CS;
  const int split = p.split > 1 ? p.split : 1;
  const int part = (int)blockIdx.x % split, bslot = (int)blockIdx.x / split;
  const int blk = p.blocks ? p.blocks[bslot] : bslot;
  const int tstride = (int)blockDim.x * split, tfirst = part * (int)blockDim.x + (int)threadIdx.x;
  double *diag = p.packed;
  double *lnk = diag + (size_t)p.K * BB;
  double *g = lnk + (size_t)p.nlinks * BB;
  double *tail = g + (size_t)p.K * B;
  if (blk < p.K)
  {
    const int k = blk;
    const int a0 = p.adj_start[k], a1 = p.adj_start[k + 1];
    constexpr int S = 2;
    for (int base = 0; base < BB + B; base += S * tstride)
    {
    double acc[S] = {0.0, 0.0};
    int bi[S], bj[S];
    bool isg[S], valid[S];
#pragma unroll
    for (int s = 0; s < S; ++s)
    {
      const int idx = base + tfirst + s * tstride;
      valid[s] = idx < BB + B;
      isg[s] = idx >= BB;
      bi[s] = isg[s] ? idx - BB : idx / B;
      bj[s] = isg[s] ? 0 : idx % B;
    }
#pragma unroll 4
    for (int a = a0; a < a1; ++a)
    {
      const AdjEntry ae = p.adj[a];
      const int lt = KP ? (ae.type & 1) : ae.type;
      const bool kp = KP && ae.type >= 2;
      const int D = lt == 0 ? Dp : Dg;
      const float *A = kp ? (lt == 0 ? p.AtA_kr : p.AtA_km) : (lt == 0 ? p.AtA_p : p.AtA_g);
      const float *b = kp ? (lt == 0 ? p.Atb_kr : p.Atb_km) : (lt == 0 ? p.Atb_p : p.Atb_g);
#pragma unroll
      for (int s = 0; s < S; ++s)
      {
        if (!valid[s])
          continue;
        const int ci = edge_col(lt, ae.role, bi[s], p.CS);
        const int cj = isg[s] ? 0 : edge_col(lt, ae.role, bj[s], p.CS);
        if (ci < 0 || cj < 0)
          continue;
        const double *Wd = kp ? nullptr : (lt == 0 ? p.wide_p : p.wide_g);
        if (Wd)
          acc[s] += Wd[(size_t)ae.edge * (D * D + D) + (isg[s] ? (size_t)D * D + ci : (size_t)ci * D + cj)];
        else
          acc[s] += isg[s] ? (double)b[(size_t)ae.edge * D + ci] : (double)A[(size_t)ae.edge * D * D + (size_t)ci * D + cj];
      }
    }
#pragma unroll
    for (int s = 0; s < S; ++s)
    {
      const int idx = base + tfirst + s * tstride;
      if (!valid[s])
        continue;
      if (isg[s])
        g[(size_t)k * B + bi[s]] = acc[s];
      else
        diag[(size_t)k * BB + idx] = acc[s];
    }
    }
  }
  else if (blk < p.K + p.nlinks)
  {
    const int l = blk - p.K;
    const LinkEdges le = p.links[l];
    for (int idx = tfirst; idx < BB; idx += tstride)
    {
      const int bi = idx / B, bj = idx % B;
      double acc = 0.0;
      {
        for (int type = 0; type < 2; ++type)
        {
          if ((type == 0 && !p.AtA_p) || (type == 1 && !p.AtA_g))
            continue;
          const int D = type == 0 ? Dp : Dg;
          const float *A = type == 0 ? p.AtA_p : p.AtA_g;
          const double *Wd = type == 0 ? p.wide_p : p.wide_g;
          const size_t ws = (size_t)D * D + D;
          int ci = edge_col(type, 0, bi, p.CS), cj = edge_col(type, 1, bj, p.CS);
          if (le.e_ab >= 0 && ci >= 0 && cj >= 0)
            acc += Wd ? Wd[(size_t)le.e_ab * ws + (size_t)ci * D + cj] : (double)A[(size_t)le.e_ab * D * D + (size_t)ci * D + cj];
          ci = edge_col(type, 1, bi, p.CS);
          cj = edge_col(type, 0, bj, p.CS);
          if (le.e_ba >= 0 && ci >= 0 && cj >= 0)
            acc += Wd ? Wd[(size_t)le.e_ba * ws + (size_t)ci * D + cj] : (double)A[(size_t)le.e_ba * D * D + (size_t)ci * D + cj];
        }
      }
      if (KP && p.link_kp_start)
        for (int a = p.link_kp_start[l]; a < p.link_kp_start[l + 1]; ++a)
        {
          const AdjEntry ae = p.link_kp[a];
          const int lt = ae.type & 1, D = lt == 0 ? Dp : Dg;
          const float *A = lt == 0 ? p.AtA_kr : p.AtA_km;
          const int ci = edge_col(lt, ae.role, bi, p.CS), cj = edge_col(lt, 1 - ae.role, bj, p.CS);
          if (ci >= 0 && cj >= 0)
            acc += (double)A[(size_t)ae.edge * D * D + (size_t)ci * D + cj];
        }
      lnk[(size_t)l * BB + idx] = acc;
    }
  }
  else
  {
    if (part != 0)
      return;
    const int wave = threadIdx.x >> 6, lane = threadIdx.x & 63;
    const bool photo = (wave & 1) == 0;
    const int which = wave >> 1;
    const float *st = photo ? p.stats_p : p.stats_g;
    const int n = photo ? p.n_edges_p : p.n_edges_g;
    double acc = 0.0;
    if (st && wave < 4)
      for (int e = lane; e < n; e += 64)
        acc += (double)st[2 * e + which];
    if (KP && p.stats_k && wave < 2)
    {
      const float *sk = p.stats_k + (photo ? 0 : 2 * (size_t)p.n_kr);
      const int nk = photo ? p.n_kr : p.n_km;
      for (int t = lane; t < nk; t += 64)
        acc += (double)sk[2 * t];
    }
    for (int off = 32; off > 0; off >>= 1)
      acc += __shfl_down(acc, off);
    if (lane == 0 && wave < 4)
    {
      tail[which * 2 + (photo ? 0 : 1)] = acc;
      if (p.tail_mirror)
        p.tail_mirror[which * 2 + (photo ? 0 : 1)] = acc;
    }
  }
}

struct WindowFinalizeParams
{
  PhotoFinalizeParams ph;
  GeoFinalizeParams ge;
  int n_p, n_g;
};

template <int CS>
__global__ __launch_bounds__(kFinalizeBlock) void window_finalize_kernel(const WindowFinalizeParams prm)
{
  constexpr int LDS = photo_finalize_lds_doubles(CS) > geo_finalize_lds_doubles(CS) ? photo_finalize_lds_doubles(CS)
                                                                                    : geo_finalize_lds_doubles(CS);
  __shared__ double s[LDS];
  const int bid = (int)blockIdx.x;
  if (bid < prm.n_g)
    geo_finalize_body<CS>(prm.ge, bid, s);
  else
    photo_finalize_body<CS>(prm.ph, bid - prm.n_g, s);
}


template <bool KP>
__global__ __launch_bounds__(1024) void error_totals_kernel(const ErrorTotalsSide ph, const ErrorTotalsSide ge, double *out,
                                                            double *mirror, double epoch, const KpTotals kp)
{
  for (int idx = threadIdx.x; idx < ph.n_edges + ge.n_edges; idx += blockDim.x)
  {
    const bool photo = idx < ph.n_edges;
    const ErrorTotalsSide &sd = photo ? ph : ge;
    const int e = photo ? idx : idx - ph.n_edges;
    const int first = sd.edge_first[e], nt = sd.edge_tiles[e];
    float se = 0.f, sn = 0.f;
    for (int t0 = 0; t0 < nt; t0 += 8)
    {
      float ve[8], vn[8];
#pragma unroll
      for (int u = 0; u < 8; ++u)
      {
        const int t = t0 + u < nt ? t0 + u : nt - 1;
        ve[u] = sd.partials[(size_t)(first + t) * sd.stride + sd.err_off];
        vn[u] = sd.partials[(size_t)(first + t) * sd.stride + sd.cnt_off];
      }
#pragma unroll
      for (int u = 0; u < 8; ++u)
        if (t0 + u < nt)
        {
          se += ve[u];
          sn += vn[u];
        }
    }
    sd.stats[2 * e + 0] = sn > 0.f ? sd.scale * se / sn : sd.fallback;
    sd.stats[2 * e + 1] = sn;
  }
  __threadfence_block();
  __syncthreads();
  const int wave = threadIdx.x >> 6, lane = threadIdx.x & 63;
  if (wave >= 4)
    return;
  const bool photo = (wave & 1) == 0;
  const int which = wave >> 1;
  const ErrorTotalsSide &sd = photo ? ph : ge;
  double acc = 0.0;
  for (int e0 = lane; e0 < sd.n_edges; e0 += 64 * 8)
  {
    float v[8];
#pragma unroll
    for (int u = 0; u < 8; ++u)
    {
      const int e = e0 + 64 * u;
      v[u] = sd.stats[2 * (e < sd.n_edges ? e : lane) + which];
    }
#pragma unroll
    for (int u = 0; u < 8; ++u)
      if (e0 + 64 * u < sd.n_edges)
        acc += (double)v[u];
  }
  if (KP && kp.stats && which == 0)
  {
    const float *sk = kp.stats + (photo ? 0 : 2 * (size_t)kp.n_kr);
    const int nk = photo ? kp.n_kr : kp.n_km;
    for (int t = lane; t < nk; t += 64)
// ... 175 lines not shown
  {
    float ms = 0.f;
    if (hipEventElapsedTime(&ms, pr.first, pr.second) == hipSuccess)
    {
      w->prof_ms[which] += ms;
      w->prof_n[which] += 1;
    }
    ev_put(w, pr.first);
    ev_put(w, pr.second);
  }
  w->pending[which].clear();
  if (total_ms)
    *total_ms = w->prof_ms[which];
  if (launches)
    *launches = w->prof_n[which];
  w->prof_ms[which] = 0;
  w->prof_n[which] = 0;
  return SAGE_OK;
}

static void upload_vars_host(SageWindow *w, int set, std::vector<float> &buf)
{
  buf.assign((size_t)w->K * w->VS, 0.f);
  const int CS = w->cfg.CS;
  for (int k = 0; k < w->K; ++k)
  {
    float *d = &buf[(size_t)k * w->VS];
    std::memcpy(d, &w->pose[set][(size_t)k * 12], 12 * sizeof(float));
    d[12] = w->scale[set][k];
    std::memcpy(d + 13, &w->code[set][(size_t)k * CS], CS * sizeof(float));
  }
}

int window_upload_vars(SageWindow *w, int set)
{
  if (w->dpt_set == set)
    w->dpt_set = -1;
  if (set == 0)
    ++w->vars_epoch;
  std::vector<float> buf;
  upload_vars_host(w, set, buf);
  SAGE_HIP(hipMemcpyAsync(w->vars[set].p, buf.data(), buf.size() * sizeof(float), hipMemcpyHostToDevice, w->stream));
  SAGE_HIP(hipStreamSynchronize(w->stream));
  return SAGE_OK;
}


static int window_launch_keypoints(SageWindow *w, int set, bool jac)
{
  const int nloc = w->n_kr + w->n_km;
  if (nloc == 0)
    return SAGE_OK;
  KpBatchParams kp{};
  kp.terms = w->kp_table.as<KpTerm>();
  kp.vars = w->vars[set].as<float>();
  kp.VS = w->VS;
  kp.cam = w->cfg.pyr.cam[0];
  kp.eps = w->cfg.eps;
  kp.AtA_r = w->AtA_kr.as<float>(); kp.Atb_r = w->Atb_kr.as<float>();
  kp.AtA_m = w->AtA_km.as<float>(); kp.Atb_m = w->Atb_km.as<float>();
  kp.stats = w->stats_k.as<float>() + (jac ? 0 : (size_t)2 * nloc);
  LaunchCommon lc{};
  prof_attach(w, jac ? 4 : 5, lc);
  if (lc.ev_start)
    (void)hipEventRecord(lc.ev_start, w->stream);
  SAGE_HIP(launch_keypoint_batch(w->stream, w->cfg.CS, jac, nloc, w->n_km > 0, kp));
  if (lc.ev_stop)
    (void)hipEventRecord(lc.ev_stop, w->stream);
  if (jac)
    w->kp_lin = true;
  return SAGE_OK;
}

extern "C" int sage_window_num_keyframes(const SageWindow *w) { return w ? w->K : 0; }
extern "C" int sage_window_num_links(const SageWindow *w) { return w ? (int)w->links.size() : 0; }
extern "C" int sage_window_block_size(const SageWindow *w) { return w ? w->B : 0; }
extern "C" size_t sage_window_packed_count(const SageWindow *w)
{
  if (!w)
    return 0;
  const size_t BB = (size_t)w->B * w->B;
  return (size_t)w->K * BB + w->links.size() * BB + (size_t)w->K * w->B + 4;
}
extern "C" double *sage_window_packed_dev(SageWindow *w) { return w ? w->packed.as<double>() : nullptr; }
extern "C" double *sage_window_error_dev(SageWindow *w) { return w ? w->errbuf.as<double>() : nullptr; }
extern "C" double sage_window_residuals_per_linearize(const SageWindow *w) { return w ? w->residuals_per_lin : 0; }
extern "C" double sage_window_bytes_per_linearize(const SageWindow *w) { return w ? w->bytes_per_lin : 0; }

int window_local_edge(const SageWindow *w, int global_edge)
{
  const auto it = std::lower_bound(w->local_edges.begin(), w->local_edges.end(), global_edge);
  return it != w->local_edges.end() && *it == global_edge ? (int)(it - w->local_edges.begin()) : -1;
}

static LaunchCommon window_lc(SageWindow *w, bool photo, bool photo_linearize = false)
{
  LaunchCommon lc{};
  lc.work = (photo ? w->work_p : w->work_g).as<WorkItem>();
  lc.edge_first = (photo ? w->first_p : w->first_g).as<int32_t>();
  lc.edge_tiles = (photo ? w->tiles_p : w->tiles_g).as<int32_t>();
  lc.n_work = photo ? w->n_work_p : w->n_work_g;
  lc.n_edges = w->n_edges;
  lc.partials = photo ? w->part_p.as<float>() : w->part_g.as<float>();
  lc.tiles_per_block = photo ? w->tpb_p : w->tpb_g;
  lc.packed = photo;
  if (photo_linearize && w->flush_p > 0)
  {
    lc.edge_first = w->rec_first_p.as<int32_t>();
    lc.edge_tiles = w->rec_count_p.as<int32_t>();
    lc.flush = w->flush_p;
  }
  return lc;
}

static AssembleParams window_assemble_params(SageWindow *w)
{
  const SageWindowConfig &c = w->cfg;
  AssembleParams ap{};
  const bool has = w->n_edges > 0;
  ap.AtA_p = (has && c.use_photo) ? w->AtA_p.as<float>() : nullptr;
  ap.Atb_p = w->Atb_p.as<float>();
  ap.stats_p = (has && c.use_photo) ? w->stats_p.as<float>() : nullptr;
  ap.AtA_g = (has && c.use_geo) ? w->AtA_g.as<float>() : nullptr;
  ap.wide_p = (has && c.use_photo) ? w->wide_p.as<double>() : nullptr;
  ap.wide_g = (has && c.use_geo) ? w->wide_g.as<double>() : nullptr;
  ap.Atb_g = w->Atb_g.as<float>();
  ap.stats_g = (has && c.use_geo) ? w->stats_g.as<float>() : nullptr;
  ap.adj_start = w->adj_start.as<int32_t>();
  ap.adj = w->adj.as<AdjEntry>();
  ap.links = w->link_edges.as<LinkEdges>();
  ap.packed = w->packed.as<double>();
  ap.tail_mirror = w->world == 1 && !w->allreduce ? w->h_err : nullptr;
  ap.K = w->K;
  ap.nlinks = (int)w->links.size();
  ap.CS = c.CS;
  ap.n_edges_p = w->n_edges;
  ap.n_edges_g = w->n_edges;
  ap.split = 1;
  ap.blocks = nullptr;
  if (w->n_kr + w->n_km > 0)
  {
    ap.AtA_kr = w->AtA_kr.as<float>(); ap.Atb_kr = w->Atb_kr.as<float>();
    ap.AtA_km = w->AtA_km.as<float>(); ap.Atb_km = w->Atb_km.as<float>();
    ap.stats_k = w->stats_k.as<float>();
    ap.link_kp_start = w->kp_link_start.as<int32_t>();
    ap.link_kp = w->kp_link.as<AdjEntry>();
    ap.n_kr = w->n_kr;
    ap.n_km = w->n_km;
  }
  return ap;
}

int window_linearize_set(SageWindow *w, int set, double *dst, bool local_blocks, bool merge)
{
  if (!w || !w->finalized)
    return SAGE_E_STATE;
  const SageWindowConfig &c = w->cfg;
  const int H = (int)c.pyr.cam[0].h, W = (int)c.pyr.cam[0].w;
  if (w->n_edges > 0)
  {
    const bool have_depth = w->dpt_set == set;
    SAGE_HIP(launch_depth_batch(w->stream, c.CS, w->depth_items[set].as<DepthItem>(), w->n_depth, H, W, !have_depth,
                                !(have_depth && w->dgrad_valid)));
    w->dpt_set = set;
    w->dgrad_valid = true;
    LaunchCommon lcg = window_lc(w, false), lcp = window_lc(w, true, true);
    lcg.stage = 1;
    lcp.stage = 1;
    merge = merge && w->merge_ok;
    lcg.merge_geo_weight = lcp.merge_geo_weight = merge ? c.geo_weight : 0.f;
    if (c.use_geo)
    {
      EdgeOut out{w->AtA_g.as<float>(), w->Atb_g.as<float>(), w->stats_g.as<float>(), w->wide_g.as<double>()};
      prof_attach(w, 1, lcg);
      SAGE_HIP(launch_geo_linearize(w->stream, c.CS, nullptr, w->gtab[set].as<GeoEdge>(), lcg, c.pyr.cam[0], c.eps,
                                    c.geo_loss_param, c.geo_weight, out));
    }
    if (c.use_photo)
    {
      EdgeOut out{w->AtA_p.as<float>(), w->Atb_p.as<float>(), w->stats_p.as<float>(), w->wide_p.as<double>()};
      prof_attach(w, 0, lcp);
      SAGE_HIP(launch_photo_linearize(w->stream, c.CS, c.FS, nullptr, w->ptab[set].as<PhotoEdge>(), lcp, c.pyr,
                                      c.photo_weights, c.eps, out));
    }
    {
      const int rck = window_launch_keypoints(w, set, true);
      if (rck)
        return rck;
    }
    WindowFinalizeParams fp{};
    fp.n_p = c.use_photo ? w->n_edges : 0;
    fp.n_g = c.use_geo ? w->n_edges : 0;
    fp.ph.table = w->ptab[set].as<PhotoEdge>();
    fp.ph.edge_first = lcp.edge_first; fp.ph.edge_tiles = lcp.edge_tiles; fp.ph.partials = lcp.partials;
    fp.ph.AtA = w->AtA_p.as<float>(); fp.ph.Atb = w->Atb_p.as<float>(); fp.ph.stats = w->stats_p.as<float>();
    fp.ph.wide = w->wide_p.as<double>();
    for (int l = 0; l < c.pyr.levels; ++l)
      fp.ph.wsum += c.photo_weights[l];
    fp.ge.table = w->gtab[set].as<GeoEdge>();
    fp.ge.edge_first = lcg.edge_first; fp.ge.edge_tiles = lcg.edge_tiles; fp.ge.partials = lcg.partials;
    fp.ge.AtA = w->AtA_g.as<float>(); fp.ge.Atb = w->Atb_g.as<float>(); fp.ge.stats = w->stats_g.as<float>();
    fp.ge.wide = w->wide_g.as<double>();
    fp.ge.weight = c.geo_weight;
    if (merge)
    {
      fp.ge.photo_partials = lcp.partials;
      fp.ge.photo_rec_first = lcp.edge_first;
      fp.ge.photo_rec_count = lcp.edge_tiles;
    }
    if (c.CS == 32)
      hipLaunchKernelGGL((window_finalize_kernel<32>), dim3(fp.n_p + fp.n_g), dim3(kFinalizeBlock), 0, w->stream, fp);
    else
      hipLaunchKernelGGL((window_finalize_kernel<16>), dim3(fp.n_p + fp.n_g), dim3(kFinalizeBlock), 0, w->stream, fp);
    SAGE_HIP(hipGetLastError());
  }
  AssembleParams ap = window_assemble_params(w);
  if (dst)
    ap.packed = dst;
  ap.split = 4;
  int nblocks = w->K + ap.nlinks + 1;
  if (local_blocks && w->n_asm_blocks > 0)
  {
    ap.blocks = w->asm_blocks.as<int32_t>();
    nblocks = w->n_asm_blocks;
  }
  if (w->n_kr + w->n_km > 0)
    hipLaunchKernelGGL(assemble_kernel<true>, dim3(nblocks * ap.split), dim3(512), 0, w->stream, ap);
  else
    hipLaunchKernelGGL(assemble_kernel<false>, dim3(nblocks * ap.split), dim3(512), 0, w->stream, ap);
  SAGE_HIP(hipGetLastError());
  window_phase_mark(w, 1);
  if (ap.packed == w->packed.as<double>())
  {
    w->have_lin = true;
    w->lin_epoch = set == 0 ? w->vars_epoch : 0;
    w->spec_err_valid = false;
    w->packed_reduced = false;
  }
  return SAGE_OK;
}

extern "C" int sage_window_linearize(SageWindow *w)
{
  if (w)
    window_phase_mark(w, 0);
  return window_linearize_set(w, 0);
}

static int window_error_pass(SageWindow *w, int which, bool speculate_gradients);
extern "C" int sage_window_error(SageWindow *w, int which) { return window_error_pass(w, which, false); }


static int window_error_pass(SageWindow *w, int which, bool speculate_gradients)
{
  if (!w || !w->finalized || which < 0 || which > 1)
    return SAGE_E_STATE;
  const SageWindowConfig &c = w->cfg;
  const int H = (int)c.pyr.cam[0].h, W = (int)c.pyr.cam[0].w;
  const bool has = w->n_edges > 0;
  if (has && w->dpt_set != which)
  {
    SAGE_HIP(launch_depth_batch(w->stream, c.CS, w->depth_items[which].as<DepthItem>(), w->n_depth, H, W, true, false));
    w->dpt_set = which;
    w->dgrad_valid = false;
  }
  ErrorTotalsSide ph{}, ge{};
  const bool fused = has && c.use_photo && c.use_geo;
  if (has && c.use_photo)
  {
    LaunchCommon lc = window_lc(w, true);
    prof_attach(w, 2, lc);
    lc.stage = 1;
    lc.fused_geo_loss_param = fused ? c.geo_loss_param : 0.f;
    SAGE_HIP(launch_photo_error(w->stream, c.CS, c.FS, nullptr, w->ptab[which].as<PhotoEdge>(), lc, c.pyr,
                                c.photo_weights, c.eps, w->stats_p.as<float>()));
    float wsum = 0.f;
    for (int l = 0; l < c.pyr.levels; ++l)
      wsum += c.photo_weights[l];
    ph = ErrorTotalsSide{lc.edge_first, lc.edge_tiles, lc.partials, w->stats_p.as<float>(), 10.0f * wsum, 1.0f, w->n_edges,
                         fused ? 4 : 2, 0, 1};
    if (fused)
      ge = ErrorTotalsSide{lc.edge_first, lc.edge_tiles, lc.partials, w->stats_g.as<float>(), 10.0f * c.geo_weight,
                           c.geo_weight, w->n_edges, 4, 2, 3};
  }
  if (has && c.use_geo && !fused)
  {
    LaunchCommon lc = window_lc(w, false);
    prof_attach(w, 3, lc);
    lc.stage = 1;
    SAGE_HIP(launch_geo_error(w->stream, c.CS, nullptr, w->gtab[which].as<GeoEdge>(), lc, c.pyr.cam[0], c.eps,
                              c.geo_loss_param, c.geo_weight, w->stats_g.as<float>()));
    ge = ErrorTotalsSide{lc.edge_first, lc.edge_tiles, lc.partials, w->stats_g.as<float>(), 10.0f * c.geo_weight,
                         c.geo_weight, w->n_edges, 2, 0, 1};
  }
  KpTotals kpt{};
  if (w->n_kr + w->n_km > 0)
  {
    const int rck = window_launch_keypoints(w, which, false);
    if (rck)
      return rck;
    kpt = KpTotals{w->stats_k.as<float>() + (size_t)2 * (w->n_kr + w->n_km), w->n_kr, w->n_km};
  }
  w->err_epoch += 1;
  double *const mirror = w->world == 1 && !w->allreduce && w->h_err ? w->h_err + 4 : nullptr;
  if (kpt.stats)
    hipLaunchKernelGGL(error_totals_kernel<true>, dim3(1), dim3(1024), 0, w->stream, ph, ge, w->errbuf.as<double>(), mirror,
                       (double)w->err_epoch, kpt);
  else
    hipLaunchKernelGGL(error_totals_kernel<false>, dim3(1), dim3(1024), 0, w->stream, ph, ge, w->errbuf.as<double>(), mirror,
                       (double)w->err_epoch, kpt);
  SAGE_HIP(hipGetLastError());
  window_phase_mark(w, 4);
  if (speculate_gradients && has && c.use_geo && w->dpt_set == which && !w->dgrad_valid)
  {
    SAGE_HIP(launch_depth_batch(w->stream, c.CS, w->depth_items[which].as<DepthItem>(), w->n_depth, H, W, false, true));
    w->dgrad_valid = true;
  }
  return SAGE_OK;
}

static int window_total_error(SageWindow *w, int from_linearize, double *err, bool stream_idle);

static bool window_spin_totals(SageWindow *w, bool reduced_mirror = false)
{
  if (!w->h_err)
    return false;
  if (!reduced_mirror && (w->world != 1 || w->allreduce || w->err_epoch == 0))
    return false;
  const volatile double *t = w->h_err + (reduced_mirror ? 12 : 8);
  const double want = (double)(reduced_mirror ? w->mirror_epoch : w->err_epoch);
  const auto t0 = std::chrono::steady_clock::now();
  unsigned spins = 0;
  while (!(t[0] == want && t[1] == want && t[2] == want && t[3] == want))
  {
    __builtin_ia32_pause();
    if ((++spins & 0x3ff) == 0 &&
        std::chrono::duration<double>(std::chrono::steady_clock::now() - t0).count() > 0.05)
      return false;
  }
  std::atomic_thread_fence(std::memory_order_acquire);
  return true;
}

static int window_allreduce(SageWindow *w, double *buf, size_t n, int iterate)
{
  if (w->allreduce && w->allreduce(buf, n, w->allreduce_user))
    return SAGE_E_STATE;
  if (w->emu_rest && w->emu_n > 0)
  {
    const size_t np = sage_window_packed_count(w);
    const double *rest = w->emu_rest + (size_t)(((iterate % w->emu_n) + w->emu_n) % w->emu_n) * np;
    if (n == np)
      hipLaunchKernelGGL(add_doubles_kernel, dim3((unsigned)((np + 255) / 256)), dim3(256), 0, w->stream, rest, buf, np);
    else if (n == 4)
      hipLaunchKernelGGL(add_doubles_kernel, dim3(1), dim3(64), 0, w->stream, rest + np - 4, buf, (size_t)4);
    else
      return SAGE_E_UNSUPPORTED;
    SAGE_HIP(hipGetLastError());
  }
  return SAGE_OK;
}

__global__ void copy_doubles_kernel(const double *__restrict__ src, double *__restrict__ dst, size_t n);
static int window_allreduce_into(SageWindow *w, const double *send, double *recv, size_t n, int iterate)
{
  if (w->allreduce2)
  {
    if (w->allreduce2(send, recv, n, w->allreduce_user))
      return SAGE_E_STATE;
    SageAllReduceFn keep = w->allreduce;
    w->allreduce = nullptr;
    const int rc = window_allreduce(w, recv, n, iterate);
    w->allreduce = keep;
    return rc;
  }
  hipLaunchKernelGGL(copy_doubles_kernel, dim3((unsigned)((n + 255) / 256)), dim3(256), 0, w->stream, send, recv, n);
  SAGE_HIP(hipGetLastError());
  return window_allreduce(w, recv, n, iterate);
}

static int window_mirror_totals(SageWindow *w, bool with_err, const double *system = nullptr)
{
  w->mirror_epoch += 1;
  hipLaunchKernelGGL(mirror_totals_kernel, dim3(1), dim3(64), 0, w->stream,
                     (system ? system : w->packed.as<double>()) + sage_window_packed_count(w) - 4,
                     with_err ? w->errbuf.as<double>() : nullptr,
                     w->h_err, (double)w->mirror_epoch);
  SAGE_HIP(hipGetLastError());
  return SAGE_OK;
}

int window_sync_candidate(SageWindow *w, bool stream_idle)
{
  if (!w->cand_pending)
    return SAGE_OK;
  if (!stream_idle)
    SAGE_HIP(hipStreamSynchronize(w->stream));
  w->cand_pending = false;
  const DeviceSolver *S = w->solver;
  if (solver_host_status(S) != 0)
    return SAGE_E_NOT_PSD;
  const int K = w->K, CS = w->cfg.CS, VS = w->VS;
  const float *v = solver_host_vars(S);
  for (int k = 0; k < K; ++k)
  {
    std::memcpy(&w->pose[1][(size_t)k * 12], v + (size_t)k * VS, 12 * sizeof(float));
    w->scale[1][k] = v[(size_t)k * VS + 12];
    std::memcpy(&w->code[1][(size_t)k * CS], v + (size_t)k * VS + 13, CS * sizeof(float));
  }
  std::memcpy(w->delta.data(), solver_host_delta(S), w->delta.size() * sizeof(double));
  return SAGE_OK;
}

static int window_wait_mirror(SageWindow *w, bool *not_psd)
{
  const bool idle = window_spin_totals(w, true);
  const int rc = window_sync_candidate(w, idle);
  if (rc && rc != SAGE_E_NOT_PSD)
    return rc;
  *not_psd = rc == SAGE_E_NOT_PSD;
  if (!idle)
    SAGE_HIP(hipStreamSynchronize(w->stream));
  return SAGE_OK;
}

static void pose_local(const float *origin, const float *other, double out[6])
{
  double Rr[9];
  for (int i = 0; i < 3; ++i)
    for (int j = 0; j < 3; ++j)
      Rr[i * 3 + j] = (double)other[i * 3 + 0] * origin[j * 3 + 0] + (double)other[i * 3 + 1] * origin[j * 3 + 1] +
                      (double)other[i * 3 + 2] * origin[j * 3 + 2];
  for (int i = 0; i < 3; ++i)
    out[i] = other[9 + i] - (Rr[i * 3 + 0] * origin[9] + Rr[i * 3 + 1] * origin[10] + Rr[i * 3 + 2] * origin[11]);
  const double tr = Rr[0] + Rr[4] + Rr[8];
  const double cs = std::min(1.0, std::max(-1.0, 0.5 * (tr - 1.0)));
  const double th = std::acos(cs);
  const double k = th < 1e-8 ? 0.5 : th / (2.0 * std::sin(th));
  out[3] = k * (Rr[7] - Rr[5]);
  out[4] = k * (Rr[2] - Rr[6]);
  out[5] = k * (Rr[3] - Rr[1]);
}

static double prior_error(const SageWindow *w, int set)
{
  const SageWindowConfig &c = w->cfg;
  double e = 0;
  for (int k = 0; k < w->K; ++k)
  {
    double s = 0;
    for (int i = 0; i < c.CS; ++i)
      s += (double)w->code[set][(size_t)k * c.CS + i] * w->code[set][(size_t)k * c.CS + i];
    e += c.code_prior_weight * s / c.CS;
  }
  if (c.scale_prior_weight > 0)
  {
    const double d = std::log((double)w->scale_init[0]) - std::log((double)w->scale[set][0]);
    e += c.scale_prior_weight * d * d;
  }
  if (c.pose_prior_weight > 0)
  {
    double loc[6];
    pose_local(&w->pose[set][0], &w->pose_init[0], loc);
    for (int i = 0; i < 6; ++i)
      e += c.pose_prior_weight * loc[i] * loc[i];
// ... 25 lines not shown
    if (!stream_idle)
      SAGE_HIP(hipStreamSynchronize(w->stream));
    *err = mirrored_error(w, from_linearize ? 0 : 4, from_linearize ? 0 : 1);
    return rc_out;
  }
  if (from_linearize)
  {
    const size_t off = sage_window_packed_count(w) - 4;
    SAGE_HIP(hipMemcpyAsync(t, w->packed.as<double>() + off, 4 * sizeof(double), hipMemcpyDeviceToHost, w->stream));
  }
  else
    SAGE_HIP(hipMemcpyAsync(t, w->errbuf.p, 4 * sizeof(double), hipMemcpyDeviceToHost, w->stream));
  SAGE_HIP(hipStreamSynchronize(w->stream));
  *err = t[0] + t[1] + prior_error(w, from_linearize ? 0 : 1);
  return rc_out;
}

static void window_priors(const SageWindow *w, std::vector<double> &dadd, std::vector<double> &gadd)
{
  const SageWindowConfig &c = w->cfg;
  const int K = w->K, B = w->B, CS = c.CS;
  dadd.assign((size_t)K * B, 0.0);
  gadd.assign((size_t)K * B, 0.0);
  for (int k = 0; k < K; ++k)
    for (int i = 0; i < CS; ++i)
    {
      dadd[k * B + 6 + i] += c.code_prior_weight;
      gadd[k * B + 6 + i] += c.code_prior_weight * (0.0 - (double)w->code[0][(size_t)k * CS + i]);
    }
  if (c.scale_prior_weight > 0)
  {
    const double s = w->scale[0][0];
    dadd[6 + CS] += c.scale_prior_weight / (s * s);
    gadd[6 + CS] += c.scale_prior_weight / s * (std::log((double)w->scale_init[0]) - std::log(s));
  }
  if (c.pose_prior_weight > 0)
  {
    double loc[6];
    pose_local(&w->pose[0][0], &w->pose_init[0], loc);
    for (int i = 0; i < 6; ++i)
    {
      dadd[i] += c.pose_prior_weight;
      gadd[i] += c.pose_prior_weight * loc[i];
    }
  }
}

static void window_retract_candidate(SageWindow *w, bool local_only)
{
  const int K = w->K, B = w->B, CS = w->cfg.CS;
  if (local_only)
  {
    w->pose[1] = w->pose[0];
    w->code[1] = w->code[0];
    w->scale[1] = w->scale[0];
  }
  for (int k = 0; k < K; ++k)
  {
    if (local_only && !sage_shard_keyframe_is_local(w->shard, k))
      continue;
    float d6[6];
    for (int i = 0; i < 6; ++i)
      d6[i] = (float)w->delta[(size_t)k * B + i];
    sage_pose_retract(&w->pose[0][(size_t)k * 12], d6, &w->pose[1][(size_t)k * 12]);
    for (int i = 0; i < CS; ++i)
      w->code[1][(size_t)k * CS + i] = w->code[0][(size_t)k * CS + i] + (float)w->delta[(size_t)k * B + 6 + i];
    w->scale[1][k] = w->scale[0][k] + (float)w->delta[(size_t)k * B + 6 + CS];
  }
}

extern "C" int sage_window_solve(SageWindow *w, double damp, double *step_norm)
{
  if (!w || !w->finalized || !w->have_lin)
    return SAGE_E_STATE;
  const SageWindowConfig &c = w->cfg;
  const int K = w->K, B = w->B, CS = c.CS;
  if (w->solver)
  {
    int rc = window_sync_candidate(w);
    if (rc && rc != SAGE_E_NOT_PSD)
      return rc;
    if (w->dpt_set == 1)
      w->dpt_set = -1;
    rc = solver_run(w->solver, w->stream, w->packed.as<double>(), w->vars[0].as<float>(), w->vars[1].as<float>(), CS,
                    damp, c.code_prior_weight, c.scale_prior_weight, c.pose_prior_weight, w->scale_init[0],
                    &w->pose_init[0]);
    if (rc)
      return rc;
    window_phase_mark(w, 3);
    w->cand_pending = true;
    if (step_norm)
    {
      if ((rc = window_sync_candidate(w)))
        return rc;
      *step_norm = std::sqrt(solver_host_step_norm2(w->solver));
    }
    return SAGE_OK;
  }
  const size_t np = sage_window_packed_count(w);
  static const bool dbg = sage::env_flag("SAGE_DEBUG_TIMING");
  auto tnow = [] { return std::chrono::steady_clock::now(); };
  auto t_a = tnow();
  SAGE_HIP(hipStreamSynchronize(w->stream));
  auto t_b = tnow();
  SAGE_HIP(hipMemcpyAsync(w->host_packed.data(), w->packed.p, np * sizeof(double), hipMemcpyDeviceToHost, w->stream));
  SAGE_HIP(hipStreamSynchronize(w->stream));
  auto t_c = tnow();
  std::vector<double> dadd, gadd;
  window_priors(w, dadd, gadd);
  std::vector<int32_t> lk(2 * w->links.size());
  for (size_t l = 0; l < w->links.size(); ++l)
  {
    lk[2 * l] = w->links[l].first;
    lk[2 * l + 1] = w->links[l].second;
  }
  int rcs = sage_block_solve(w->host_packed.data(), K, (int)w->links.size(), lk.data(), B, damp, dadd.data(),
                             gadd.data(), w->delta.data());
  if (rcs)
    return rcs;
  auto t_d = tnow();
  double nrm = 0;
  for (double v : w->delta)
    nrm += v * v;
  if (step_norm)
    *step_norm = std::sqrt(nrm);
  window_retract_candidate(w, false);
  const int rcu = window_upload_vars(w, 1);
  if (dbg)
  {
    auto t_e = tnow();
    auto ms = [](auto a, auto b) { return std::chrono::duration<double, std::milli>(b - a).count(); };
    fprintf(stderr, "[sage solve] wait-kernels %.3f d2h %.3f block_solve %.3f retract+h2d %.3f ms\n", ms(t_a, t_b),
            ms(t_b, t_c), ms(t_c, t_d), ms(t_d, t_e));
  }
  return rcu;
}

extern "C" int sage_window_accept(SageWindow *w)
{
  if (!w || !w->finalized)
    return SAGE_E_STATE;
  int rcs = window_sync_candidate(w);
  if (rcs)
    return rcs;
  w->pose[0] = w->pose[1];
  w->code[0] = w->code[1];
  w->scale[0] = w->scale[1];
  ++w->vars_epoch;
  ++w->emu_cur;
  w->dpt_set = w->dpt_set == 1 ? 0 : -1;
  const int nv = w->K * w->VS;
  hipLaunchKernelGGL(copy_floats_kernel, dim3((nv + 255) / 256), dim3(256), 0, w->stream, w->vars[1].as<float>(),
                     w->vars[0].as<float>(), nv);
  SAGE_HIP(hipGetLastError());
  return SAGE_OK;
}

extern "C" int sage_window_reset(SageWindow *w)
{
  if (!w || !w->finalized)
    return SAGE_E_STATE;
  (void)window_sync_candidate(w);
  for (int s = 0; s < 2; ++s)
  {
    w->pose[s] = w->pose_init;
    w->code[s] = w->code_added;
    w->scale[s] = w->scale_init;
  }
  int rc;
  if ((rc = window_upload_vars(w, 0)) || (rc = window_upload_vars(w, 1)))
    return rc;
  w->have_lin = false;
  w->emu_cur = 0;
  return SAGE_OK;
}

extern "C" int sage_window_get_keyframe(const SageWindow *w, int kf, float *pose12, float *code, float *scale)
{
  if (!w || kf < 0 || kf >= w->K)
    return SAGE_E_INVALID;
  if (pose12)
    std::memcpy(pose12, &w->pose[0][(size_t)kf * 12], 12 * sizeof(float));
// ... 235 lines not shown
  const bool sharded = w->allreduce != nullptr;
  if (seq == LmSeq::schur)
  {
    double lin_error = 0;
    if ((rc = schur_solve(w, st->damp, &lin_error)) && rc != SAGE_E_NOT_PSD)
      return rc;
    window_phase_mark(w, 3);
    if (first)
      st->error = lin_error;
    st->candidate_error = INFINITY;
    if (rc == SAGE_E_NOT_PSD)
      return SAGE_OK;
    if ((rc = sage_window_error(w, 1)))
      return rc;
    hipLaunchKernelGGL(add_to_double_kernel, dim3(1), dim3(1), 0, w->stream, w->errbuf.as<double>(),
                       prior_error_owned(w, 1));
    if (w->allreduce(w->errbuf.as<double>(), 4, w->allreduce_user))
      return SAGE_E_STATE;
    double t4[4];
    SAGE_HIP(hipMemcpyAsync(t4, w->errbuf.p, sizeof(t4), hipMemcpyDeviceToHost, w->stream));
    SAGE_HIP(hipStreamSynchronize(w->stream));
    st->candidate_error = t4[0] + t4[1];
    return SAGE_OK;
  }
  rc = sage_window_solve(w, st->damp, nullptr);
  if (rc == SAGE_E_NOT_PSD)
  {
    st->candidate_error = INFINITY;
    return first && seq == LmSeq::classic ? sage_window_total_error(w, 1, &st->error) : SAGE_OK;
  }
  if (rc)
    return rc;
  if (seq == LmSeq::at_candidate)
  {
    std::memcpy(ev.cur_tot, w->h_err, sizeof(ev.cur_tot));
    ev.have_cur_tot = true;
    bool not_psd;
    if ((rc = window_form_system(w, 1, w->packed_save.as<double>(), w->emu_cur + 1)) ||
        (rc = window_wait_mirror(w, &not_psd)))
      return rc;
    st->candidate_error = not_psd ? INFINITY : mirrored_error(w, 0, 1);
    return SAGE_OK;
  }
  if ((rc = window_error_pass(w, 1, !sharded)))
    return rc;
  if (!sharded)
  {
    const bool idle = window_spin_totals(w);
    if (first && (rc = window_total_error(w, 1, &st->error, idle)))
      return rc;
    if ((rc = window_total_error(w, 0, &st->candidate_error, idle)) == SAGE_E_NOT_PSD)
      st->candidate_error = INFINITY;
    return rc == SAGE_E_NOT_PSD ? SAGE_OK : rc;
  }
  bool not_psd;
  if ((rc = window_allreduce(w, w->errbuf.as<double>(), 4, w->emu_cur + 1)) || (rc = window_mirror_totals(w, true)) ||
      (rc = window_wait_mirror(w, &not_psd)))
    return rc;
  if (first)
    st->error = mirrored_error(w, 0, 0);
  st->candidate_error = not_psd ? INFINITY : mirrored_error(w, 4, 1);
  return SAGE_OK;
}

static int lm_accept(LmSeq seq, SageWindow *w, const SageLmState *st)
{
  const int rc = sage_window_accept(w);
  if (rc || seq != LmSeq::at_candidate)
    return rc;
  std::swap(w->packed.p, w->packed_save.p);
  std::swap(w->packed.cap, w->packed_save.cap);
  w->lin_epoch = w->vars_epoch;
  w->packed_reduced = true;
  w->spec_error = st->candidate_error;
  return SAGE_OK;
}

static void lm_reject(SageWindow *w, const LmEval &ev)
{
  if (ev.have_cur_tot)
    std::memcpy(w->h_err, ev.cur_tot, sizeof(ev.cur_tot));
}

extern "C" int sage_window_lm_step(SageWindow *w, SageLmState *st, const SageLmConfig *cfg)
{
  if (!w || !st || !cfg)
    return SAGE_E_INVALID;
  if (w->world > 1 && !w->allreduce)
    return SAGE_E_STATE;
  const LmSeq seq = lm_sequence_for(w, cfg);
  auto clampd = [&](double d) { return std::min(std::max((double)cfg->min_damp, d), (double)cfg->max_damp); };
  if (st->iters == 0 && st->damp <= 0)
    st->damp = cfg->init_damp;
  window_phase_mark(w, 0);
  int rc = lm_prepare(seq, w, st);
  if (rc)
    return rc;
  st->accepted = 0;
  for (int evals = 1;; ++evals)
  {
    LmEval ev{};
    if ((rc = lm_evaluate(seq, w, st, evals == 1, ev)))
      return rc;
    if (st->candidate_error < st->error)
    {
      st->accepted = 1;
      if ((rc = lm_accept(seq, w, st)))
        return rc;
      st->damp = clampd(st->damp / cfg->damp_dec_factor);
      break;
    }
    lm_reject(w, ev);
    const bool give_up = st->damp >= cfg->max_damp || (cfg->max_inner_evals > 0 && evals >= cfg->max_inner_evals);
    st->damp = clampd(st->damp * cfg->damp_inc_factor);
    if (give_up)
      break;
  }
  st->iters += 1;
  return SAGE_OK;
}

static int window_lm_run(SageWindow *w, SageLmState *st, const SageLmConfig *cfg, int n, double *trace, int *done,
                         double *step_seconds)
{
  if (!w || !st || !cfg || n < 0)
    return SAGE_E_INVALID;
  int i = 0, rc = SAGE_OK;
  auto t_prev = std::chrono::steady_clock::now();
  for (; i < n; ++i)
  {
    if ((rc = sage_window_lm_step(w, st, cfg)))
      break;
    if (trace)
    {
      trace[4 * i + 0] = st->error;
      trace[4 * i + 1] = st->candidate_error;
      trace[4 * i + 2] = (double)st->accepted;
      trace[4 * i + 3] = st->damp;
    }
    if (step_seconds)
    {
      const auto t = std::chrono::steady_clock::now();
      step_seconds[i] = std::chrono::duration<double>(t - t_prev).count();
      t_prev = t;
    }
  }
  if (done)
    *done = i;
  return rc;
}

extern "C" int sage_window_lm_run(SageWindow *w, SageLmState *st, const SageLmConfig *cfg, int n, double *trace, int *done)
{
  return window_lm_run(w, st, cfg, n, trace, done, nullptr);
}

extern "C" int sage_window_lm_run_timed(SageWindow *w, SageLmState *st, const SageLmConfig *cfg, int n, double *trace,
                                        int *done, double *step_seconds)
{
  return window_lm_run(w, st, cfg, n, trace, done, step_seconds);
}
```

sage_slam_amd/csrc/window_build.hip:

```cpp
#include "runtime_internal.h"
#include "window_plan.h"

static std::atomic<int> g_live_windows{0};

extern "C" int sage_window_create(const SageWindowConfig *cfg, void *hip_stream, SageWindow **out)
{
  if (!cfg || !out || !cfg->mask_dev)
    return SAGE_E_INVALID;
  if (!supported(cfg->CS, cfg->FS) || cfg->pyr.levels < 1 || cfg->pyr.levels > SAGE_MAX_LEVELS)
    return SAGE_E_UNSUPPORTED;
  int ndev = 0;
  SAGE_HIP(hipGetDeviceCount(&ndev));
  if (ndev < 1)
    return (int)hipErrorNoDevice;
  SageWindow *w = new SageWindow();
  w->cfg = *cfg;
  w->stream = reinterpret_cast<hipStream_t>(hip_stream);
  w->B = 7 + cfg->CS;
  w->VS = ((13 + cfg->CS + 3) / 4) * 4;
  *out = w;
  g_live_windows.fetch_add(1, std::memory_order_acq_rel);
  return SAGE_OK;
}

// ... 579 lines not shown
  int rc;
  int tpb_g = plan::geo_run(plan::total_tiles(tiles));
  if (const char *e = getenv("SAGE_GEO_TPB"))
    tpb_g = std::max(1, atoi(e));
  WorkList wl;
  wl.build(fs.Nedge, tpb_g);
  w->n_work_g = (int)wl.work.size();
  w->tpb_g = wl.tiles_per_block;
  if ((rc = upload(w->work_g, wl.work, w->stream)) || (rc = upload(w->first_g, wl.edge_first, w->stream)) ||
      (rc = upload(w->tiles_g, wl.edge_tiles, w->stream)))
    return rc;
  SAGE_HIP(hipStreamSynchronize(w->stream));
  int tpb = plan::photo_run(tiles, w->cfg.FS);
  if (const char *e = getenv("SAGE_PHOTO_TPB"))
    tpb = std::max(1, atoi(e));
  w->Nedge = fs.Nedge;
  w->tpb_heur = tpb;
  if ((rc = window_plan_photo_runs(w, tpb, photo_flush_for_runs(tpb))))
    return rc;
  SAGE_HIP(hipStreamSynchronize(w->stream));
  return SAGE_OK;
}

static int finalize_results(SageWindow *w, const FinalizeState &fs)
{
  const int CS = w->cfg.CS, K = w->K;
  int rc;
  const size_t Dp = 13 + CS, Dg = 14 + 2 * CS;
  const size_t ne = std::max(1, w->n_edges);
  if ((rc = w->part_p.reserve(std::max<size_t>(1, std::max(w->n_work_p, w->n_rec_p)) * photo_partial_floats(CS) * sizeof(float))) ||
      (rc = w->part_g.reserve(std::max<size_t>(1, w->n_work_g) * geo_partial_floats(CS) * sizeof(float))) ||
      (rc = w->AtA_p.reserve(ne * Dp * Dp * sizeof(float))) || (rc = w->Atb_p.reserve(ne * Dp * sizeof(float))) ||
      (rc = w->stats_p.reserve(ne * 2 * sizeof(float))) || (rc = w->AtA_g.reserve(ne * Dg * Dg * sizeof(float))) ||
      (rc = w->Atb_g.reserve(ne * Dg * sizeof(float))) || (rc = w->stats_g.reserve(ne * 2 * sizeof(float))))
    return rc;
  if ((rc = w->wide_p.reserve(ne * (Dp * Dp + Dp) * sizeof(double))) ||
      (rc = w->wide_g.reserve(ne * (Dg * Dg + Dg) * sizeof(double))))
    return rc;
  std::vector<int32_t> adj_start(K + 1, 0);
  std::vector<AdjEntry> adj;
  for (int k = 0; k < K; ++k)
  {
    adj_start[k] = (int32_t)adj.size();
    adj.insert(adj.end(), fs.adjv[k].begin(), fs.adjv[k].end());
  }
  adj_start[K] = (int32_t)adj.size();
  if ((rc = upload(w->adj_start, adj_start, w->stream)) || (rc = upload(w->adj, adj, w->stream)) ||
      (rc = upload(w->link_edges, fs.le, w->stream)))
    return rc;
  SAGE_HIP(hipStreamSynchronize(w->stream));
  if ((rc = w->packed.reserve(sage_window_packed_count(w) * sizeof(double))) || (rc = w->errbuf.reserve(4 * sizeof(double))))
    return rc;
  {
    std::vector<int32_t> ids;
    for (int k = 0; k < K; ++k)
      if (!fs.adjv[k].empty())
        ids.push_back(k);
    for (size_t l = 0; l < fs.le.size(); ++l)
      if (fs.le[l].e_ab >= 0 || fs.le[l].e_ba >= 0)
        ids.push_back(K + (int32_t)l);
    ids.push_back(K + (int32_t)w->links.size());
    w->n_asm_blocks = (int)ids.size();
    if ((rc = upload(w->asm_blocks, ids, w->stream)))
      return rc;
    SAGE_HIP(hipStreamSynchronize(w->stream));
  }
  SAGE_HIP(hipMemsetAsync(w->packed.p, 0, sage_window_packed_count(w) * sizeof(double), w->stream));
  SAGE_HIP(hipMemsetAsync(w->errbuf.p, 0, 4 * sizeof(double), w->stream));
  if (!w->h_err)
  {
    SAGE_HIP(hipHostMalloc(reinterpret_cast<void **>(&w->h_err), 16 * sizeof(double), hipHostMallocDefault));
    std::memset(w->h_err, 0, 16 * sizeof(double));
  }
  w->host_packed.assign(sage_window_packed_count(w), 0.0);
  w->delta.assign((size_t)K * w->B, 0.0);
  return SAGE_OK;
}

static int finalize_solver(SageWindow *w, const FinalizeState &fs)
{
  int rc = solver_create(&w->solver, w->K, w->B, w->VS, w->links, w->stream);
  if (rc != SAGE_OK && rc != SAGE_E_UNSUPPORTED)
    return rc;
  if (!fs.domain_solve)
    return SAGE_OK;
  std::vector<int32_t> lk(2 * w->links.size());
  for (size_t l = 0; l < w->links.size(); ++l)
  {
    lk[2 * l] = w->links[l].first;
    lk[2 * l + 1] = w->links[l].second;
  }
  if ((rc = sage_shard_plan_create(w->K, (int)w->links.size(), lk.data(), w->B, w->rank, w->world, &w->shard)))
    return rc;
  const size_t ns = sage_shard_sep_count(w->shard);
  w->h_sep.assign(ns, 0.0);
  if ((rc = w->sepbuf.reserve(ns * sizeof(double))))
    return rc;
  w->host_packed.resize(sage_window_packed_count(w));
  return SAGE_OK;
}

extern "C" int sage_window_finalize(SageWindow *w)
{
  if (!w || w->finalized || w->K < 1)
    return SAGE_E_INVALID;
  FinalizeState fs;
  const char *schur = getenv("SAGE_SHARD_SCHUR");
  fs.domain_solve = plan::uses_domain_solve(w->world, w->K, schur ? atoi(schur) != 0 : -1);
  int rc;
  if ((rc = finalize_variables(w)) || (rc = finalize_ownership(w, fs)) || (rc = finalize_pyramids(w)) ||
      (rc = finalize_samples(w)) || (rc = finalize_source_features(w, fs)) || (rc = finalize_edge_tables(w, fs)) ||
      (rc = window_finalize_keypoints(w, fs.adjv, &fs.residuals)))
    return rc;
  w->residuals_per_lin = fs.residuals;
  w->bytes_per_lin = fs.bytes;
  if ((rc = finalize_work_lists(w, fs)) || (rc = finalize_results(w, fs)) || (rc = finalize_solver(w, fs)))
    return rc;
  w->finalized = true;
  if (const char *e = getenv("SAGE_AUTOTUNE"))
    if (atoi(e) != 0)
      return sage_window_tune_runs(w, nullptr, nullptr, nullptr, nullptr);
  return SAGE_OK;
}

extern "C" int sage_window_set_runs(SageWindow *w, int tpb)
{
  if (!w || !w->finalized)
    return SAGE_E_STATE;
  if (tpb < 1 || tpb > 64)
    return SAGE_E_INVALID;
  return window_plan_photo_runs(w, tpb, photo_flush_for_runs(tpb));
}

extern "C" int sage_window_tune_runs(SageWindow *w, int *tpb_out, int *tpb_rule_out, float *ms_rule_out, float *ms_best_out)
{
  if (!w || !w->finalized)
    return SAGE_E_STATE;
  const int rule = w->tpb_heur;
  if (tpb_out)
    *tpb_out = w->tpb_p;
  if (tpb_rule_out)
    *tpb_rule_out = rule;
  if (ms_rule_out)
    *ms_rule_out = 0.f;
  if (ms_best_out)
    *ms_best_out = 0.f;
  if (getenv("SAGE_PHOTO_TPB") || w->world > 1 || w->allreduce || w->n_edges == 0 || !(w->cfg.use_photo))
    return SAGE_OK;
  const std::vector<int> cand = plan::tune_candidates(rule, plan::typical_edge(edge_tiles(w->Nedge)));
  const bool prof_was = w->profiling;
  const int level_was = w->prof_level;
  int rc = sage_window_set_profiling(w, 1);
  double best_ms = 0.0, rule_ms = 0.0;
  int best = rule;
  auto measure = [&](int t, double &ms) -> int {
    int r = window_plan_photo_runs(w, t, photo_flush_for_runs(t));
    for (int rep = 0; rep < 4 && !r; ++rep)
    {
      if ((r = sage_window_linearize(w)) || (r = sage_window_error(w, 1)))
        break;
      double lin = 0.0, err = 0.0;
      int nl = 0, ne = 0;
      if ((r = sage_window_get_kernel_time(w, 0, &lin, &nl)) || (r = sage_window_get_kernel_time(w, 2, &err, &ne)))
        break;
      const double tt = lin / std::max(1, nl) + err / std::max(1, ne);
      if (rep > 0)
// ... 44 lines not shown
```

Before: 255,200 Mresiduals/s.

## Defer Hessian assembly and fuse it into the device solver launch

Assembly of the packed normal-equation system is deferred during classic LM steps on a single device, and instead performed inside the device solver (solver_run_assembling), which assembles directly from per-edge AtA/Atb. This is meant to remove a separate assemble kernel launch and the round trip through the packed buffer before the solve. Every other consumer of the packed buffer (packed_dev, mirror totals, host solve path) flushes the pending assembly first to stay correct. It adds state tracking and a risk of stale data if some path misses the flush; an env flag disables it.

```diff
diff --git a/include/sage_ba.h b/include/sage_ba.h
--- a/include/sage_ba.h
+++ b/include/sage_ba.h
@@ -115,6 +115,8 @@
 
 int sage_block_solve(const double *packed_host, int K, int nlinks, const int32_t *links, int B, double damp,
                      const double *diag_add, const double *g_add, double *delta);
+int sage_block_plan_link_cover(int K, int nlinks, const int32_t *links, int32_t *cover, int32_t *bad_sources,
+                               int32_t *fill_blocks);
 long long sage_solve_lookahead_count(void);
 
 typedef struct SageLmConfig
@@ -356,6 +358,7 @@
 int sage_window_lm_run(SageWindow *w, SageLmState *st, const SageLmConfig *cfg, int n, double *trace, int *done);
 int sage_window_lm_run_timed(SageWindow *w, SageLmState *st, const SageLmConfig *cfg, int n, double *trace, int *done,
                              double *step_seconds);
+int sage_window_fused_tail_launches(const SageWindow *w);
 int sage_window_sync_variables(SageWindow *w);
 
 #ifdef __cplusplus
diff --git a/sage_slam_amd/build.py b/sage_slam_amd/build.py
--- a/sage_slam_amd/build.py
+++ b/sage_slam_amd/build.py
@@ -12,7 +12,7 @@
 LIB = os.path.join(HERE, "libsage_ba.so")
 SOURCES = ["photo_kernels.hip", "geo_kernels.hip", "track_kernels.hip", "producers.hip", "keypoint_kernels.hip", "solve_kernels.hip", "operators.hip", "tracker.hip", "window.hip", "window_build.hip", "window_dist.hip", "window_factors.hip",
            "host_math.cpp", "block_solver.cpp", "host_threads.cpp", "shard_solve.cpp"]
-HEADERS = ["sage_device.h", "sage_internal.h", "host_math.h", "block_solver.h", "host_threads.h", "runtime_internal.h", "finalize_bodies.h", "keypoint_batch.h", "window_plan.h", os.path.join(ROOT, "include", "sage_ba.h")]
+HEADERS = ["sage_device.h", "sage_internal.h", "host_math.h", "block_solver.h", "host_threads.h", "runtime_internal.h", "finalize_bodies.h", "assemble_bodies.h", "scatter_bodies.h", "keypoint_batch.h", "window_plan.h", os.path.join(ROOT, "include", "sage_ba.h")]
 HIPCC = os.environ.get("HIPCC", "/opt/rocm/bin/hipcc")
 HOSTCXX = os.environ.get("HOSTCXX", "/opt/rocm/lib/llvm/bin/clang++")
 FLAGS = ["--offload-arch=gfx950", "-O3", "-std=c++17", "-fPIC", "-Wall", "-Wno-unused-function",
diff --git a/sage_slam_amd/capi.py b/sage_slam_amd/capi.py
--- a/sage_slam_amd/capi.py
+++ b/sage_slam_amd/capi.py
@@ -92,14 +92,14 @@
     "sage_tracker_photo_jac_error_calculate", "sage_tracker_photo_error_calculate",
     "sage_geometric_jac_error_calculate", "sage_geometric_error_calculate", "sage_depth_and_grad",
     "sage_gaussian_pyramid_with_grad", "sage_se3_exp", "sage_pose_retract", "sage_nearest_psd", "sage_nearest_psd_reference", "sage_factor_block_count", "sage_factor_hessian_blocks",
-    "sage_damped_solve_qr_f32", "sage_block_solve", "sage_solve_lookahead_count", "sage_lm_config_default", "sage_track_lm", "sage_track_frame",
+    "sage_damped_solve_qr_f32", "sage_block_solve", "sage_block_plan_link_cover", "sage_solve_lookahead_count", "sage_lm_config_default", "sage_track_lm", "sage_track_frame",
     "sage_window_create", "sage_window_destroy", "sage_window_add_keyframe", "sage_window_add_link", "sage_window_set_link_geo_loss",
     "sage_window_set_shard", "sage_window_finalize", "sage_window_num_keyframes", "sage_window_num_links",
     "sage_window_block_size", "sage_window_packed_count", "sage_window_packed_dev",
     "sage_window_residuals_per_linearize", "sage_window_bytes_per_linearize", "sage_window_linearize",
     "sage_window_error", "sage_window_tune_runs", "sage_window_set_runs", "sage_window_error_dev", "sage_window_solve", "sage_window_total_error",
     "sage_window_accept", "sage_window_reset", "sage_window_get_keyframe", "sage_window_set_keyframe", "sage_window_get_delta",
-    "sage_window_get_edge", "sage_window_add_keypoint_term", "sage_window_num_keypoint_terms", "sage_window_get_keypoint_term", "sage_window_prepass", "sage_window_factor", "sage_window_factor_error", "sage_window_prepare_factors", "sage_factor_psd", "sage_factor_cut_blocks", "sage_window_set_profiling", "sage_window_get_kernel_time", "sage_window_get_phase_time", "sage_window_lm_step", "sage_window_lm_run", "sage_window_lm_run_timed", "sage_window_sync_variables", "sage_window_set_allreduce", "sage_shard_plan_create", "sage_shard_plan_create_domains", "sage_block_solve_domains", "sage_shard_plan_destroy", "sage_shard_sep_count", "sage_shard_num_separators", "sage_shard_num_interior", "sage_shard_keyframe_owner", "sage_shard_keyframe_is_local", "sage_shard_eliminate", "sage_shard_solve", "sage_rccl_unique_id", "sage_rccl_comm_create", "sage_rccl_comm_destroy", "sage_rccl_comm_info", "sage_window_use_rccl", "sage_window_emulate_peers", "sage_sort_locations", "sage_bind_thread_to_device", "sage_solver_helper_cpus", "sage_solver_placement_moves", "sage_placement_monitor", "sage_shutdown", "sage_host_threads_running",
+    "sage_window_get_edge", "sage_window_add_keypoint_term", "sage_window_num_keypoint_terms", "sage_window_get_keypoint_term", "sage_window_prepass", "sage_window_factor", "sage_window_factor_error", "sage_window_prepare_factors", "sage_factor_psd", "sage_factor_cut_blocks", "sage_window_set_profiling", "sage_window_get_kernel_time", "sage_window_get_phase_time", "sage_window_lm_step", "sage_window_lm_run", "sage_window_lm_run_timed", "sage_window_fused_tail_launches", "sage_window_sync_variables", "sage_window_set_allreduce", "sage_shard_plan_create", "sage_shard_plan_create_domains", "sage_block_solve_domains", "sage_shard_plan_destroy", "sage_shard_sep_count", "sage_shard_num_separators", "sage_shard_num_interior", "sage_shard_keyframe_owner", "sage_shard_keyframe_is_local", "sage_shard_eliminate", "sage_shard_solve", "sage_rccl_unique_id", "sage_rccl_comm_create", "sage_rccl_comm_destroy", "sage_rccl_comm_info", "sage_window_use_rccl", "sage_window_emulate_peers", "sage_sort_locations", "sage_bind_thread_to_device", "sage_solver_helper_cpus", "sage_solver_placement_moves", "sage_placement_monitor", "sage_shutdown", "sage_host_threads_running",
     "sage_valid_locations", "sage_shuffle_indices", "sage_sample_locations",
     "sage_reprojection_jac_error_calculate", "sage_reprojection_error_calculate",
     "sage_tracker_reproj_jac_error_calculate", "sage_tracker_reproj_error_calculate",
@@ -229,6 +229,16 @@
                                 C.c_double(damp), dp(da), dp(ga), delta.ctypes.data_as(C.POINTER(C.c_double))),
          "sage_block_solve")
     return delta
+
+
+def block_plan_link_cover(K, links):
+    lk = np.ascontiguousarray(np.asarray(links, dtype=np.int32).reshape(-1))
+    cover = np.zeros(len(lk) // 2, np.int32)
+    bad, fill = C.c_int32(), C.c_int32()
+    _chk(lib().sage_block_plan_link_cover(K, len(lk) // 2, lk.ctypes.data_as(C.POINTER(C.c_int32)),
+                                          cover.ctypes.data_as(C.POINTER(C.c_int32)), C.byref(bad), C.byref(fill)),
+         "sage_block_plan_link_cover")
+    return cover, bad.value, fill.value
 
 
 def solve_lookahead_count() -> int:
@@ -652,6 +662,9 @@
                                             C.byref(done), sec.ctypes.data_as(C.POINTER(C.c_double))), "sage_window_lm_run_timed")
         return tr[:done.value], sec[:done.value]
 
+    def fused_tail_launches(self) -> int:
+        return int(lib().sage_window_fused_tail_launches(self.h))
+
     def delta(self):
         d = np.zeros(self.K * self.B, np.float64)
         _chk(lib().sage_window_get_delta(self.h, d.ctypes.data_as(C.POINTER(C.c_double))), "sage_window_get_delta")
diff --git a/sage_slam_amd/csrc/assemble_bodies.h b/sage_slam_amd/csrc/assemble_bodies.h
--- /dev/null
+++ b/sage_slam_amd/csrc/assemble_bodies.h
@@ -0,0 +1,180 @@
+#pragma once
+
+#include <hip/hip_runtime.h>
+#include <stdint.h>
+
+namespace sage
+{
+struct AdjEntry
+{
+  int32_t type;
+  int32_t edge;
+  int32_t role;
+};
+
+struct LinkEdges
+{
+  int32_t e_ab, e_ba;
+};
+
+struct AssembleParams
+{
+  const float *AtA_p, *Atb_p, *stats_p;
+  const float *AtA_g, *Atb_g, *stats_g;
+  const double *wide_p, *wide_g;
+  const int32_t *adj_start;
+  const AdjEntry *adj;
+  const LinkEdges *links;
+  double *packed;
+  double *tail_mirror;
+  int K, nlinks, CS, n_edges_p, n_edges_g;
+  int split;
+  const int32_t *blocks;
+  const float *AtA_kr, *Atb_kr, *AtA_km, *Atb_km, *stats_k;
+  const int32_t *link_kp_start;
+  const AdjEntry *link_kp;
+  int n_kr, n_km;
+};
+
+struct DeviceSolver;
+bool solver_can_assemble(const DeviceSolver *S);
+int solver_run_assembling(DeviceSolver *S, hipStream_t stream, const AssembleParams &ap, bool keypoint_terms,
+                          const float *vars0, float *vars1, double damp, double code_w, double scale_w, double pose_w,
+                          float scale_init0, const float *pose_init0);
+
+#if defined(__HIPCC__)
+__device__ __forceinline__ int edge_col(int type, int role, int bi, int CS)
+{
+  if (bi < 6)
+    return role * 6 + bi;
+  if (type == 0)
+  {
+    if (role == 1)
+      return -1;
+    return bi < 6 + CS ? 12 + (bi - 6) : 12 + CS;
+  }
+  if (bi < 6 + CS)
+    return 12 + role * CS + (bi - 6);
+  return 12 + 2 * CS + role;
+}
+
+template <bool KP, class Put>
+__device__ __forceinline__ void assemble_keyframe_sums(const AssembleParams &p, int k, int tfirst, int tstride, Put put)
+{
+  const int B = 7 + p.CS, BB = B * B;
+  const int Dp = 13 + p.CS, Dg = 14 + 2 * p.CS;
+  const int a0 = p.adj_start[k], a1 = p.adj_start[k + 1];
+  constexpr int S = 2;
+  for (int base = 0; base < BB + B; base += S * tstride)
+  {
+    double acc[S] = {0.0, 0.0};
+    int bi[S], bj[S];
+    bool isg[S], valid[S];
+#pragma unroll
+    for (int s = 0; s < S; ++s)
+    {
+      const int idx = base + tfirst + s * tstride;
+      valid[s] = idx < BB + B;
+      isg[s] = idx >= BB;
+      bi[s] = isg[s] ? idx - BB : idx / B;
+      bj[s] = isg[s] ? 0 : idx % B;
+    }
+#pragma unroll 4
+    for (int a = a0; a < a1; ++a)
+    {
+      const AdjEntry ae = p.adj[a];
+      const int lt = KP ? (ae.type & 1) : ae.type;
+      const bool kp = KP && ae.type >= 2;
+      const int D = lt == 0 ? Dp : Dg;
+      const float *A = kp ? (lt == 0 ? p.AtA_kr : p.AtA_km) : (lt == 0 ? p.AtA_p : p.AtA_g);
+      const float *b = kp ? (lt == 0 ? p.Atb_kr : p.Atb_km) : (lt == 0 ? p.Atb_p : p.Atb_g);
+#pragma unroll
+      for (int s = 0; s < S; ++s)
+      {
+        if (!valid[s])
+          continue;
+        const int ci = edge_col(lt, ae.role, bi[s], p.CS);
+        const int cj = isg[s] ? 0 : edge_col(lt, ae.role, bj[s], p.CS);
+        if (ci < 0 || cj < 0)
+          continue;
+        const double *Wd = kp ? nullptr : (lt == 0 ? p.wide_p : p.wide_g);
+        if (Wd)
+          acc[s] += Wd[(size_t)ae.edge * (D * D + D) + (isg[s] ? (size_t)D * D + ci : (size_t)ci * D + cj)];
+        else
+          acc[s] += isg[s] ? (double)b[(size_t)ae.edge * D + ci] : (double)A[(size_t)ae.edge * D * D + (size_t)ci * D + cj];
+      }
+    }
+#pragma unroll
+    for (int s = 0; s < S; ++s)
+      if (valid[s])
+        put(base + tfirst + s * tstride, acc[s]);
+  }
+}
+
+template <bool KP>
+__device__ __forceinline__ double assemble_link_element(const AssembleParams &p, int l, const LinkEdges le, int idx)
+{
+  const int B = 7 + p.CS;
+  const int Dp = 13 + p.CS, Dg = 14 + 2 * p.CS;
+  const int bi = idx / B, bj = idx % B;
+  double acc = 0.0;
+  for (int type = 0; type < 2; ++type)
+  {
+    if ((type == 0 && !p.AtA_p) || (type == 1 && !p.AtA_g))
+      continue;
+    const int D = type == 0 ? Dp : Dg;
+    const float *A = type == 0 ? p.AtA_p : p.AtA_g;
+    const double *Wd = type == 0 ? p.wide_p : p.wide_g;
+    const size_t ws = (size_t)D * D + D;
+    int ci = edge_col(type, 0, bi, p.CS), cj = edge_col(type, 1, bj, p.CS);
+    if (le.e_ab >= 0 && ci >= 0 && cj >= 0)
+      acc += Wd ? Wd[(size_t)le.e_ab * ws + (size_t)ci * D + cj] : (double)A[(size_t)le.e_ab * D * D + (size_t)ci * D + cj];
+    ci = edge_col(type, 1, bi, p.CS);
+    cj = edge_col(type, 0, bj, p.CS);
+    if (le.e_ba >= 0 && ci >= 0 && cj >= 0)
+      acc += Wd ? Wd[(size_t)le.e_ba * ws + (size_t)ci * D + cj] : (double)A[(size_t)le.e_ba * D * D + (size_t)ci * D + cj];
+  }
+  if (KP && p.link_kp_start)
+    for (int a = p.link_kp_start[l]; a < p.link_kp_start[l + 1]; ++a)
+    {
+      const AdjEntry ae = p.link_kp[a];
+      const int lt = ae.type & 1, D = lt == 0 ? Dp : Dg;
+      const float *A = lt == 0 ? p.AtA_kr : p.AtA_km;
+      const int ci = edge_col(lt, ae.role, bi, p.CS), cj = edge_col(lt, 1 - ae.role, bj, p.CS);
+      if (ci >= 0 && cj >= 0)
+        acc += (double)A[(size_t)ae.edge * D * D + (size_t)ci * D + cj];
+    }
+  return acc;
+}
+
+template <bool KP>
+__device__ __forceinline__ void assemble_tail_totals(const AssembleParams &p, double *tail)
+{
+  const int wave = threadIdx.x >> 6, lane = threadIdx.x & 63;
+  const bool photo = (wave & 1) == 0;
+  const int which = wave >> 1;
+  const float *st = photo ? p.stats_p : p.stats_g;
+  const int n = photo ? p.n_edges_p : p.n_edges_g;
+  double acc = 0.0;
+  if (st && wave < 4)
+    for (int e = lane; e < n; e += 64)
+      acc += (double)st[2 * e + which];
+  if (KP && p.stats_k && wave < 2)
+  {
+    const float *sk = p.stats_k + (photo ? 0 : 2 * (size_t)p.n_kr);
+    const int nk = photo ? p.n_kr : p.n_km;
+    for (int t = lane; t < nk; t += 64)
+      acc += (double)sk[2 * t];
+  }
+  for (int off = 32; off > 0; off >>= 1)
+    acc += __shfl_down(acc, off);
+  if (lane == 0 && wave < 4)
+  {
+    tail[which * 2 + (photo ? 0 : 1)] = acc;
+    if (p.tail_mirror)
+      p.tail_mirror[which * 2 + (photo ? 0 : 1)] = acc;
+  }
+}
+#endif
+
+}
diff --git a/sage_slam_amd/csrc/block_solver.cpp b/sage_slam_amd/csrc/block_solver.cpp
--- a/sage_slam_amd/csrc/block_solver.cpp
+++ b/sage_slam_amd/csrc/block_solver.cpp
@@ -1598,6 +1598,58 @@
   env.col_ptr = plan.col_ptr.data(); env.col_rows = plan.col_rows.data();
   return env;
 }
+
+void plan_link_cover(const BlockPlan &plan, int nlinks, std::vector<int32_t> &cover, int *bad_sources)
+{
+  cover.assign((size_t)std::max(nlinks, 0), 0);
+  int bad = 0;
+  for (int b = 0; b < plan.nblk; ++b)
+  {
+    const int srcf = plan.blk_src[b];
+    if (srcf < 0)
+      continue;
+    const int src = srcf & 0x3fffffff;
+    if (plan.blk_row[b] == plan.blk_col[b] || src >= nlinks)
+      ++bad;
+    else
+      ++cover[src];
+  }
+  if (bad_sources)
+    *bad_sources = bad;
+}
+
+bool plan_links_stored_once(const BlockPlan &plan, int nlinks)
+{
+  std::vector<int32_t> cover;
+  int bad = 0;
+  plan_link_cover(plan, nlinks, cover, &bad);
+  return bad == 0 && std::all_of(cover.begin(), cover.end(), [](int32_t c) { return c == 1; });
+}
+}
+
+extern "C" int sage_block_plan_link_cover(int K, int nlinks, const int32_t *links, int32_t *cover, int32_t *bad_sources,
+                                          int32_t *fill_blocks)
+{
+  if (K < 1 || nlinks < 0 || (nlinks > 0 && !links) || !cover)
+    return SAGE_E_INVALID;
+  std::vector<std::pair<int, int>> lk(nlinks);
+  for (int l = 0; l < nlinks; ++l)
+    lk[l] = {links[2 * l], links[2 * l + 1]};
+  sage::BlockPlan bp;
+  const int rc = sage::plan_blocks(K, lk, !sage::env_flag("SAGE_SOLVE_NO_SPLIT"), bp);
+  if (rc != SAGE_OK)
+    return rc;
+  std::vector<int32_t> cv;
+  int bad = 0, fill = 0;
+  sage::plan_link_cover(bp, nlinks, cv, &bad);
+  std::copy(cv.begin(), cv.end(), cover);
+  for (int b = 0; b < bp.nblk; ++b)
+    fill += bp.blk_src[b] < 0 && bp.blk_row[b] != bp.blk_col[b];
+  if (bad_sources)
+    *bad_sources = bad;
+  if (fill_blocks)
+    *fill_blocks = fill;
+  return SAGE_OK;
 }
 
 extern "C" long long sage_solve_lookahead_count(void) { return sage::g_lookahead_count.load(); }
diff --git a/sage_slam_amd/csrc/block_solver.h b/sage_slam_amd/csrc/block_solver.h
--- a/sage_slam_amd/csrc/block_solver.h
+++ b/sage_slam_amd/csrc/block_solver.h
@@ -80,4 +80,6 @@
 };
 int plan_blocks(int K, const std::vector<std::pair<int, int>> &links, bool allow_split, BlockPlan &out);
 BlockEnvelope envelope_of(const BlockPlan &plan, int Bp);
+void plan_link_cover(const BlockPlan &plan, int nlinks, std::vector<int32_t> &cover, int *bad_sources);
+bool plan_links_stored_once(const BlockPlan &plan, int nlinks);
 }
diff --git a/sage_slam_amd/csrc/runtime_internal.h b/sage_slam_amd/csrc/runtime_internal.h
--- a/sage_slam_amd/csrc/runtime_internal.h
+++ b/sage_slam_amd/csrc/runtime_internal.h
@@ -36,6 +36,7 @@
 #include "sage_ba.h"
 #include "sage_internal.h"
 #include "keypoint_batch.h"
+#include "assemble_bodies.h"
 
 using namespace sage;
 
@@ -153,37 +154,6 @@
 
 namespace sage
 {
-struct AdjEntry
-{
-  int32_t type;
-  int32_t edge;
-  int32_t role;
-};
-
-struct LinkEdges
-{
-  int32_t e_ab, e_ba;
-};
-
-struct AssembleParams
-{
-  const float *AtA_p, *Atb_p, *stats_p;
-  const float *AtA_g, *Atb_g, *stats_g;
-  const double *wide_p, *wide_g;
-  const int32_t *adj_start;
-  const AdjEntry *adj;
-  const LinkEdges *links;
-  double *packed;
-  double *tail_mirror;
-  int K, nlinks, CS, n_edges_p, n_edges_g;
-  int split;
-  const int32_t *blocks;
-  const float *AtA_kr, *Atb_kr, *AtA_km, *Atb_km, *stats_k;
-  const int32_t *link_kp_start;
-  const AdjEntry *link_kp;
-  int n_kr, n_km;
-};
-
 struct KpTotals
 {
   const float *stats;
@@ -256,6 +226,8 @@
   std::vector<double> delta;
   sage::DeviceSolver *solver = nullptr;
   bool cand_pending = false;
+  bool fuse_tail = false, asm_defer = false, asm_pending = false;
+  int fused_tail_launches = 0;
   double residuals_per_lin = 0, bytes_per_lin = 0;
   bool have_lin = false;
   uint64_t vars_epoch = 1, lin_epoch = 0;
diff --git a/sage_slam_amd/csrc/scatter_bodies.h b/sage_slam_amd/csrc/scatter_bodies.h
--- /dev/null
+++ b/sage_slam_amd/csrc/scatter_bodies.h
@@ -0,0 +1,117 @@
+#pragma once
+
+#include <hip/hip_runtime.h>
+#include <stdint.h>
+
+namespace sage
+{
+
+struct SolvePlan
+{
+  int K, B, Bp, nblk, nlinks;
+  const int32_t *row_first;
+  const int32_t *row_off;
+  const int32_t *blk_row, *blk_col, *blk_src;
+  const int32_t *perm, *pos;
+};
+
+struct SolvePriors
+{
+  double code_w, scale_w, pose_w;
+  float scale_init0;
+  float pose_init0[12];
+};
+
+#if defined(__HIPCC__)
+__device__ inline void pose_local_dev(const float *origin, const float *other, double out[6])
+{
+  double Rr[9];
+  for (int i = 0; i < 3; ++i)
+    for (int j = 0; j < 3; ++j)
+      Rr[i * 3 + j] = (double)other[i * 3 + 0] * origin[j * 3 + 0] + (double)other[i * 3 + 1] * origin[j * 3 + 1] +
+                      (double)other[i * 3 + 2] * origin[j * 3 + 2];
+  for (int i = 0; i < 3; ++i)
+    out[i] = other[9 + i] - (Rr[i * 3 + 0] * origin[9] + Rr[i * 3 + 1] * origin[10] + Rr[i * 3 + 2] * origin[11]);
+  const double tr = Rr[0] + Rr[4] + Rr[8];
+  const double cs = fmin(1.0, fmax(-1.0, 0.5 * (tr - 1.0)));
+  const double th = acos(cs);
+  const double k = th < 1e-8 ? 0.5 : th / (2.0 * sin(th));
+  out[3] = k * (Rr[7] - Rr[5]);
+  out[4] = k * (Rr[2] - Rr[6]);
+  out[5] = k * (Rr[3] - Rr[1]);
+}
+
+__device__ __forceinline__ void scatter_block_priors(int tid, int B, int CS, int kf, const float *var, const SolvePriors &pri,
+                                                     double *s_dadd, double *s_gadd)
+{
+  if (tid < B)
+  {
+    double da = 0.0, ga = 0.0;
+    if (tid >= 6 && tid < 6 + CS)
+    {
+      da = pri.code_w;
+      ga = pri.code_w * (0.0 - (double)var[13 + tid - 6]);
+    }
+    if (kf == 0 && tid == 6 + CS && pri.scale_w > 0)
+    {
+      const double s = (double)var[12];
+      da = pri.scale_w / (s * s);
+      ga = pri.scale_w / s * (log((double)pri.scale_init0) - log(s));
+    }
+    if (kf == 0 && tid < 6 && pri.pose_w > 0)
+    {
+      double loc[6];
+      pose_local_dev(var, pri.pose_init0, loc);
+      da = pri.pose_w;
+      ga = pri.pose_w * loc[tid];
+    }
+    s_dadd[tid] = da;
+    s_gadd[tid] = ga;
+  }
+}
+
+__device__ __forceinline__ void scatter_store_block(int tid, int nthreads, int B, int Bp, bool is_diag, bool has_src, bool flip,
+                                                    int transposed, const double *diag, const double *lnk,
+                                                    const double *s_dadd, double damp, double *__restrict__ out)
+{
+  for (int o = tid; o < Bp * Bp; o += nthreads)
+  {
+    const int hi = o / Bp, lo = o - hi * Bp;
+    const int r = transposed ? lo : hi, c = transposed ? hi : lo;
+    double v = 0.0;
+    if (is_diag)
+    {
+      if (r < B && c < B)
+      {
+        v = 0.5 * (diag[r * B + c] + diag[c * B + r]);
+        if (r == c)
+          v = (v + s_dadd[r]) * (1.0 + damp);
+      }
+      else if (r == c)
+        v = 1.0 + damp;
+    }
+    else if (has_src && r < B && c < B)
+      v = flip ? lnk[r * B + c] : lnk[c * B + r];
+    out[o] = v;
+  }
+}
+
+__device__ __forceinline__ void scatter_store_rhs(int tid, int nthreads, int B, int Bp, const double *g, const double *s_gadd,
+                                                  double *__restrict__ yrow)
+{
+  for (int r = tid; r < Bp; r += nthreads)
+    yrow[r] = r < B ? g[r] + s_gadd[r] : 0.0;
+}
+
+__device__ __forceinline__ void scatter_post_ticket(int tid, unsigned *flag, unsigned epoch)
+{
+  __syncthreads();
+  if (tid == 0)
+  {
+    __threadfence_system();
+    *reinterpret_cast<volatile unsigned *>(flag) = epoch;
+  }
+}
+#endif
+
+}
diff --git a/sage_slam_amd/csrc/solve_kernels.hip b/sage_slam_amd/csrc/solve_kernels.hip
--- a/sage_slam_amd/csrc/solve_kernels.hip
+++ b/sage_slam_amd/csrc/solve_kernels.hip
@@ -6,47 +6,15 @@
 #include <cstring>
 #include <vector>
 
+#include "assemble_bodies.h"
 #include "block_solver.h"
 #include "host_math.h"
+#include "scatter_bodies.h"
 #include "sage_device.h"
 #include "sage_internal.h"
 
 namespace sage
 {
-
-struct SolvePlan
-{
-  int K, B, Bp, nblk, nlinks;
-  const int32_t *row_first;
-  const int32_t *row_off;
-  const int32_t *blk_row, *blk_col, *blk_src;
-  const int32_t *perm, *pos;
-};
-
-struct SolvePriors
-{
-  double code_w, scale_w, pose_w;
-  float scale_init0;
-  float pose_init0[12];
-};
-
-__device__ inline void pose_local_dev(const float *origin, const float *other, double out[6])
-{
-  double Rr[9];
-  for (int i = 0; i < 3; ++i)
-    for (int j = 0; j < 3; ++j)
-      Rr[i * 3 + j] = (double)other[i * 3 + 0] * origin[j * 3 + 0] + (double)other[i * 3 + 1] * origin[j * 3 + 1] +
-                      (double)other[i * 3 + 2] * origin[j * 3 + 2];
-  for (int i = 0; i < 3; ++i)
-    out[i] = other[9 + i] - (Rr[i * 3 + 0] * origin[9] + Rr[i * 3 + 1] * origin[10] + Rr[i * 3 + 2] * origin[11]);
-  const double tr = Rr[0] + Rr[4] + Rr[8];
-  const double cs = fmin(1.0, fmax(-1.0, 0.5 * (tr - 1.0)));
-  const double th = acos(cs);
-  const double k = th < 1e-8 ? 0.5 : th / (2.0 * sin(th));
-  out[3] = k * (Rr[7] - Rr[5]);
-  out[4] = k * (Rr[2] - Rr[6]);
-  out[5] = k * (Rr[3] - Rr[1]);
-}
 
 __global__ __launch_bounds__(256) void solve_scatter_kernel(const SolvePlan P, const double *__restrict__ packed,
                                                             const float *__restrict__ vars0, int VS, int CS,
@@ -70,70 +38,81 @@
     const double *diag = packed + (size_t)kf * BB;
     const double *lnk = packed + (size_t)P.K * BB + (size_t)(src < 0 ? 0 : src) * BB;
     const double *g = packed + (size_t)P.K * BB + (size_t)P.nlinks * BB + (size_t)kf * B;
-    double *out = L + (size_t)b * Bp * Bp;
     if (i == j)
     {
-      const float *var = vars0 + (size_t)kf * VS;
-      if (tid < B)
-      {
-        double da = 0.0, ga = 0.0;
-        if (tid >= 6 && tid < 6 + CS)
-        {
-          da = pri.code_w;
-          ga = pri.code_w * (0.0 - (double)var[13 + tid - 6]);
-        }
-        if (kf == 0 && tid == 6 + CS && pri.scale_w > 0)
-        {
-          const double s = (double)var[12];
-          da = pri.scale_w / (s * s);
-          ga = pri.scale_w / s * (log((double)pri.scale_init0) - log(s));
-        }
-        if (kf == 0 && tid < 6 && pri.pose_w > 0)
-        {
-          double loc[6];
-          pose_local_dev(var, pri.pose_init0, loc);
-          da = pri.pose_w;
-          ga = pri.pose_w * loc[tid];
-        }
-        s_dadd[tid] = da;
-        s_gadd[tid] = ga;
-      }
+      scatter_block_priors(tid, B, CS, kf, vars0 + (size_t)kf * VS, pri, s_dadd, s_gadd);
       __syncthreads();
     }
-    for (int o = tid; o < Bp * Bp; o += blockDim.x)
-    {
-      const int hi = o / Bp, lo = o - hi * Bp;
-      const int r = transposed ? lo : hi, c = transposed ? hi : lo;
-      double v = 0.0;
-      if (i == j)
-      {
-        if (r < B && c < B)
-        {
-          v = 0.5 * (diag[r * B + c] + diag[c * B + r]);
-          if (r == c)
-            v = (v + s_dadd[r]) * (1.0 + damp);
-        }
-        else if (r == c)
-          v = 1.0 + damp;
-      }
-      else if (src >= 0 && r < B && c < B)
-        v = flip ? lnk[r * B + c] : lnk[c * B + r];
-      out[o] = v;
-    }
+    scatter_store_block(tid, (int)blockDim.x, B, Bp, i == j, src >= 0, flip, transposed, diag, lnk, s_dadd, damp,
+                        L + (size_t)b * Bp * Bp);
     if (i == j)
-      for (int r = tid; r < Bp; r += blockDim.x)
-        y[(size_t)i * Bp + r] = r < B ? g[r] + s_gadd[r] : 0.0;
+      scatter_store_rhs(tid, (int)blockDim.x, B, Bp, g, s_gadd, y + (size_t)i * Bp);
     if (flags)
-    {
-      __syncthreads();
-      if (tid == 0)
-      {
-        __threadfence_system();
-        *reinterpret_cast<volatile unsigned *>(flags + b) = epoch;
-      }
-    }
+      scatter_post_ticket(tid, flags + b, epoch);
     else
       __syncthreads();
+  }
+}
+
+constexpr int kFusedMaxThreads = 512;
+constexpr int kFusedWgs = 32, kFusedThreads = 512;
+constexpr int kFusedBlockDoubles = 39 * 39 + 39;
+
+template <bool KP>
+__global__ __launch_bounds__(kFusedMaxThreads) void assemble_scatter_kernel(const SolvePlan P, const AssembleParams p,
+                                                                const float *__restrict__ vars0, int VS,
+                                                                const SolvePriors pri, double damp,
+                                                                double *__restrict__ L, double *__restrict__ y,
+                                                                const int32_t *__restrict__ order, unsigned *flags,
+                                                                unsigned epoch)
+{
+  const int tid = threadIdx.x, nt = (int)blockDim.x;
+  const int B = P.B, Bp = P.Bp, BB = B * B;
+  __shared__ double s_blk[kFusedBlockDoubles];
+  __shared__ double s_dadd[64], s_gadd[64];
+  double *diag = p.packed;
+  double *lnk = diag + (size_t)P.K * BB;
+  double *g = lnk + (size_t)P.nlinks * BB;
+  for (int it = blockIdx.x; it <= P.nblk; it += gridDim.x)
+  {
+    if (it == P.nblk)
+    {
+      assemble_tail_totals<KP>(p, g + (size_t)P.K * B);
+      continue;
+    }
+    const int b = order[it];
+    const int i = P.blk_row[b], j = P.blk_col[b], srcf = P.blk_src[b];
+    const int src = srcf < 0 ? -1 : (srcf & 0x3fffffff);
+    const bool flip = srcf >= 0 && (srcf & 0x40000000);
+    if (src < 0 && i != j)
+      continue;
+    const int kf = P.perm[i];
+    if (i == j)
+    {
+      assemble_keyframe_sums<KP>(p, kf, tid, nt, [&](int idx, double v) {
+        s_blk[idx] = v;
+        if (idx >= BB)
+          g[(size_t)kf * B + idx - BB] = v;
+        else
+          diag[(size_t)kf * BB + idx] = v;
+      });
+      scatter_block_priors(tid, B, p.CS, kf, vars0 + (size_t)kf * VS, pri, s_dadd, s_gadd);
+    }
+    else
+    {
+      const LinkEdges le = p.links[src];
+      for (int idx = tid; idx < BB; idx += nt)
+      {
+        const double v = assemble_link_element<KP>(p, src, le, idx);
+        s_blk[idx] = v;
+        lnk[(size_t)src * BB + idx] = v;
+      }
+    }
+    __syncthreads();
+    scatter_store_block(tid, nt, B, Bp, i == j, src >= 0, flip, 1, s_blk, s_blk, s_dadd, damp, L + (size_t)b * Bp * Bp);
+    if (i == j)
+      scatter_store_rhs(tid, nt, B, Bp, s_blk + BB, s_gadd, y + (size_t)i * Bp);
+    scatter_post_ticket(tid, flags + b, epoch);
   }
 }
 
@@ -276,6 +255,8 @@
   unsigned *h_flags = nullptr;
   unsigned epoch = 0;
   int scatter_wgs = 32;
+  bool fusable = false;
+  int fused_wgs = kFusedWgs, fused_threads = kFusedThreads;
   std::vector<uint8_t> h_fill;
 };
 
@@ -371,6 +352,11 @@
     S->h_fill[b] = (blk_src[b] < 0 && blk_row[b] != blk_col[b]) ? 1 : 0;
   if (const char *e = getenv("SAGE_SCATTER_WGS"))
     S->scatter_wgs = std::max(1, atoi(e));
+  S->fusable = plan_links_stored_once(bp, (int)links.size()) && B * B + B <= kFusedBlockDoubles;
+  if (const char *e = getenv("SAGE_FUSED_WGS"))
+    S->fused_wgs = std::max(1, atoi(e));
+  if (const char *e = getenv("SAGE_FUSED_THREADS"))
+    S->fused_threads = std::min(kFusedMaxThreads, std::max(256, atoi(e) / 64 * 64));
   std::memset(S->h_pinned, 0, S->h_bytes);
   S->host_plan = std::move(bp);
   *out = S;
@@ -392,10 +378,17 @@
   delete S;
 }
 
-int solver_run(DeviceSolver *S, hipStream_t stream, const double *packed_dev, const float *vars0, float *vars1,
-               int CS, double damp, double code_w, double scale_w, double pose_w, float scale_init0,
-               const float *pose_init0)
-{
+bool solver_can_assemble(const DeviceSolver *S)
+{
+  return S && S->fusable && !sage::env_flag("SAGE_SCATTER_FILL");
+}
+
+static int solver_run_impl(DeviceSolver *S, hipStream_t stream, const double *packed_dev, const AssembleParams *fused,
+                           bool fused_kp, const float *vars0, float *vars1, int CS, double damp, double code_w,
+                           double scale_w, double pose_w, float scale_init0, const float *pose_init0)
+{
+  if (fused && (!solver_can_assemble(S) || fused->K != S->K || fused->nlinks != S->nlinks || 7 + fused->CS != S->B))
+    return SAGE_E_STATE;
   SolvePriors pri{};
   pri.code_w = code_w; pri.scale_w = scale_w; pri.pose_w = pose_w; pri.scale_init0 = scale_init0;
   for (int i = 0; i < 12; ++i)
@@ -410,10 +403,23 @@
     S->epoch += 1;
     if (S->epoch == 0)
       S->epoch = 1;
-    hipLaunchKernelGGL(solve_scatter_kernel, dim3(std::min(S->scatter_wgs, S->nblk)), dim3(256), 0, stream, S->plan,
-                       packed_dev, vars0, S->VS, CS, pri, damp, 1, reinterpret_cast<double *>(S->h_T),
-                       reinterpret_cast<double *>(S->h_y), S->d_order, S->h_flags, S->epoch, 0, S->nblk,
-                       sage::env_flag("SAGE_SCATTER_FILL") ? 1 : 0);
+    if (fused)
+    {
+      const dim3 grid(std::min(S->fused_wgs, S->nblk + 1)), block(S->fused_threads);
+      if (fused_kp)
+        hipLaunchKernelGGL(assemble_scatter_kernel<true>, grid, block, 0, stream, S->plan, *fused, vars0, S->VS, pri, damp,
+                           reinterpret_cast<double *>(S->h_T), reinterpret_cast<double *>(S->h_y), S->d_order, S->h_flags,
+                           S->epoch);
+      else
+        hipLaunchKernelGGL(assemble_scatter_kernel<false>, grid, block, 0, stream, S->plan, *fused, vars0, S->VS, pri, damp,
+                           reinterpret_cast<double *>(S->h_T), reinterpret_cast<double *>(S->h_y), S->d_order, S->h_flags,
+                           S->epoch);
+    }
+    else
+      hipLaunchKernelGGL(solve_scatter_kernel, dim3(std::min(S->scatter_wgs, S->nblk)), dim3(256), 0, stream, S->plan,
+                         packed_dev, vars0, S->VS, CS, pri, damp, 1, reinterpret_cast<double *>(S->h_T),
+                         reinterpret_cast<double *>(S->h_y), S->d_order, S->h_flags, S->epoch, 0, S->nblk,
+                         sage::env_flag("SAGE_SCATTER_FILL") ? 1 : 0);
     if ((eh = hipGetLastError()) != hipSuccess)
       return (int)eh;
     char *hp = reinterpret_cast<char *>(S->h_pinned);
@@ -456,6 +462,22 @@
   return SAGE_OK;
 }
 
+int solver_run(DeviceSolver *S, hipStream_t stream, const double *packed_dev, const float *vars0, float *vars1,
+               int CS, double damp, double code_w, double scale_w, double pose_w, float scale_init0,
+               const float *pose_init0)
+{
+  return solver_run_impl(S, stream, packed_dev, nullptr, false, vars0, vars1, CS, damp, code_w, scale_w, pose_w, scale_init0,
+                         pose_init0);
+}
+
+int solver_run_assembling(DeviceSolver *S, hipStream_t stream, const AssembleParams &ap, bool keypoint_terms,
+                          const float *vars0, float *vars1, double damp, double code_w, double scale_w, double pose_w,
+                          float scale_init0, const float *pose_init0)
+{
+  return solver_run_impl(S, stream, ap.packed, &ap, keypoint_terms, vars0, vars1, ap.CS, damp, code_w, scale_w, pose_w,
+                         scale_init0, pose_init0);
+}
+
 const float *solver_host_vars(const DeviceSolver *S) { return reinterpret_cast<const float *>(reinterpret_cast<const char *>(S->h_pinned) + S->h_vars_off); }
 const double *solver_host_delta(const DeviceSolver *S) { return reinterpret_cast<const double *>(reinterpret_cast<const char *>(S->h_pinned) + S->h_delta_off); }
 double solver_host_step_norm2(const DeviceSolver *S) { return *reinterpret_cast<const double *>(reinterpret_cast<const char *>(S->h_pinned) + S->h_tail_off); }
diff --git a/sage_slam_amd/csrc/window.hip b/sage_slam_amd/csrc/window.hip
--- a/sage_slam_amd/csrc/window.hip
+++ b/sage_slam_amd/csrc/window.hip
@@ -4,29 +4,10 @@
 namespace sage
 {
 
-
-
-
-__device__ __forceinline__ int edge_col(int type, int role, int bi, int CS)
-{
-  if (bi < 6)
-    return role * 6 + bi;
-  if (type == 0)
-  {
-    if (role == 1)
-      return -1;
-    return bi < 6 + CS ? 12 + (bi - 6) : 12 + CS;
-  }
-  if (bi < 6 + CS)
-    return 12 + role * CS + (bi - 6);
-  return 12 + 2 * CS + role;
-}
-
 template <bool KP>
 __global__ __launch_bounds__(1024) void assemble_kernel(const AssembleParams p)
 {
   const int B = 7 + p.CS, BB = B * B;
-  const int Dp = 13 + p.CS, Dg = 14 + 2 * p.CS;
   const int split = p.split > 1 ? p.split : 1;
   const int part = (int)blockIdx.x % split, bslot = (int)blockIdx.x / split;
   const int blk = p.blocks ? p.blocks[bslot] : bslot;
@@ -38,128 +19,22 @@
   if (blk < p.K)
   {
     const int k = blk;
-    const int a0 = p.adj_start[k], a1 = p.adj_start[k + 1];
-    constexpr int S = 2;
-    for (int base = 0; base < BB + B; base += S * tstride)
-    {
-    double acc[S] = {0.0, 0.0};
-    int bi[S], bj[S];
-    bool isg[S], valid[S];
-#pragma unroll
-    for (int s = 0; s < S; ++s)
-    {
-      const int idx = base + tfirst + s * tstride;
-      valid[s] = idx < BB + B;
-      isg[s] = idx >= BB;
-      bi[s] = isg[s] ? idx - BB : idx / B;
-      bj[s] = isg[s] ? 0 : idx % B;
-    }
-#pragma unroll 4
-    for (int a = a0; a < a1; ++a)
-    {
-      const AdjEntry ae = p.adj[a];
-      const int lt = KP ? (ae.type & 1) : ae.type;
-      const bool kp = KP && ae.type >= 2;
-      const int D = lt == 0 ? Dp : Dg;
-      const float *A = kp ? (lt == 0 ? p.AtA_kr : p.AtA_km) : (lt == 0 ? p.AtA_p : p.AtA_g);
-      const float *b = kp ? (lt == 0 ? p.Atb_kr : p.Atb_km) : (lt == 0 ? p.Atb_p : p.Atb_g);
-#pragma unroll
-      for (int s = 0; s < S; ++s)
-      {
-        if (!valid[s])
-          continue;
-        const int ci = edge_col(lt, ae.role, bi[s], p.CS);
-        const int cj = isg[s] ? 0 : edge_col(lt, ae.role, bj[s], p.CS);
-        if (ci < 0 || cj < 0)
-          continue;
-        const double *Wd = kp ? nullptr : (lt == 0 ? p.wide_p : p.wide_g);
-        if (Wd)
-          acc[s] += Wd[(size_t)ae.edge * (D * D + D) + (isg[s] ? (size_t)D * D + ci : (size_t)ci * D + cj)];
-        else
-          acc[s] += isg[s] ? (double)b[(size_t)ae.edge * D + ci] : (double)A[(size_t)ae.edge * D * D + (size_t)ci * D + cj];
-      }
-    }
-#pragma unroll
-    for (int s = 0; s < S; ++s)
-    {
-      const int idx = base + tfirst + s * tstride;
-      if (!valid[s])
-        continue;
-      if (isg[s])
-        g[(size_t)k * B + bi[s]] = acc[s];
+    assemble_keyframe_sums<KP>(p, k, tfirst, tstride, [&](int idx, double v) {
+      if (idx >= BB)
+        g[(size_t)k * B + idx - BB] = v;
       else
-        diag[(size_t)k * BB + idx] = acc[s];
-    }
-    }
+        diag[(size_t)k * BB + idx] = v;
+    });
   }
   else if (blk < p.K + p.nlinks)
   {
     const int l = blk - p.K;
     const LinkEdges le = p.links[l];
     for (int idx = tfirst; idx < BB; idx += tstride)
-    {
-      const int bi = idx / B, bj = idx % B;
-      double acc = 0.0;
-      {
-        for (int type = 0; type < 2; ++type)
-        {
-          if ((type == 0 && !p.AtA_p) || (type == 1 && !p.AtA_g))
-            continue;
-          const int D = type == 0 ? Dp : Dg;
-          const float *A = type == 0 ? p.AtA_p : p.AtA_g;
-          const double *Wd = type == 0 ? p.wide_p : p.wide_g;
-          const size_t ws = (size_t)D * D + D;
-          int ci = edge_col(type, 0, bi, p.CS), cj = edge_col(type, 1, bj, p.CS);
-          if (le.e_ab >= 0 && ci >= 0 && cj >= 0)
-            acc += Wd ? Wd[(size_t)le.e_ab * ws + (size_t)ci * D + cj] : (double)A[(size_t)le.e_ab * D * D + (size_t)ci * D + cj];
-          ci = edge_col(type, 1, bi, p.CS);
-          cj = edge_col(type, 0, bj, p.CS);
-          if (le.e_ba >= 0 && ci >= 0 && cj >= 0)
-            acc += Wd ? Wd[(size_t)le.e_ba * ws + (size_t)ci * D + cj] : (double)A[(size_t)le.e_ba * D * D + (size_t)ci * D + cj];
-        }
-      }
-      if (KP && p.link_kp_start)
-        for (int a = p.link_kp_start[l]; a < p.link_kp_start[l + 1]; ++a)
-        {
-          const AdjEntry ae = p.link_kp[a];
-          const int lt = ae.type & 1, D = lt == 0 ? Dp : Dg;
-          const float *A = lt == 0 ? p.AtA_kr : p.AtA_km;
-          const int ci = edge_col(lt, ae.role, bi, p.CS), cj = edge_col(lt, 1 - ae.role, bj, p.CS);
-          if (ci >= 0 && cj >= 0)
-            acc += (double)A[(size_t)ae.edge * D * D + (size_t)ci * D + cj];
-        }
-      lnk[(size_t)l * BB + idx] = acc;
-    }
-  }
-  else
-  {
-    if (part != 0)
-      return;
-    const int wave = threadIdx.x >> 6, lane = threadIdx.x & 63;
-    const bool photo = (wave & 1) == 0;
-    const int which = wave >> 1;
-    const float *st = photo ? p.stats_p : p.stats_g;
-    const int n = photo ? p.n_edges_p : p.n_edges_g;
-    double acc = 0.0;
-    if (st && wave < 4)
-      for (int e = lane; e < n; e += 64)
-        acc += (double)st[2 * e + which];
-    if (KP && p.stats_k && wave < 2)
-    {
-      const float *sk = p.stats_k + (photo ? 0 : 2 * (size_t)p.n_kr);
-      const int nk = photo ? p.n_kr : p.n_km;
-      for (int t = lane; t < nk; t += 64)
-        acc += (double)sk[2 * t];
-    }
-    for (int off = 32; off > 0; off >>= 1)
-      acc += __shfl_down(acc, off);
-    if (lane == 0 && wave < 4)
-    {
-      tail[which * 2 + (photo ? 0 : 1)] = acc;
-      if (p.tail_mirror)
-        p.tail_mirror[which * 2 + (photo ? 0 : 1)] = acc;
-    }
-  }
+      lnk[(size_t)l * BB + idx] = assemble_link_element<KP>(p, l, le, idx);
+  }
+  else if (part == 0)
+    assemble_tail_totals<KP>(p, tail);
 }
 
 struct WindowFinalizeParams
@@ -501,7 +376,14 @@
   const size_t BB = (size_t)w->B * w->B;
   return (size_t)w->K * BB + w->links.size() * BB + (size_t)w->K * w->B + 4;
 }
-extern "C" double *sage_window_packed_dev(SageWindow *w) { return w ? w->packed.as<double>() : nullptr; }
+static int window_flush_assembly(SageWindow *w);
+extern "C" double *sage_window_packed_dev(SageWindow *w)
+{
+  if (w)
+    (void)window_flush_assembly(w);
+  return w ? w->packed.as<double>() : nullptr;
+}
+extern "C" int sage_window_fused_tail_launches(const SageWindow *w) { return w ? w->fused_tail_launches : 0; }
 extern "C" double *sage_window_error_dev(SageWindow *w) { return w ? w->errbuf.as<double>() : nullptr; }
 extern "C" double sage_window_residuals_per_linearize(const SageWindow *w) { return w ? w->residuals_per_lin : 0; }
 extern "C" double sage_window_bytes_per_linearize(const SageWindow *w) { return w ? w->bytes_per_lin : 0; }
@@ -570,6 +452,26 @@
   return ap;
 }
 
+static void window_launch_assemble(SageWindow *w, const AssembleParams &ap, int nblocks)
+{
+  if (w->n_kr + w->n_km > 0)
+    hipLaunchKernelGGL(assemble_kernel<true>, dim3(nblocks * ap.split), dim3(512), 0, w->stream, ap);
+  else
+    hipLaunchKernelGGL(assemble_kernel<false>, dim3(nblocks * ap.split), dim3(512), 0, w->stream, ap);
+}
+
+static int window_flush_assembly(SageWindow *w)
+{
+  if (!w->asm_pending)
+    return SAGE_OK;
+  w->asm_pending = false;
+  AssembleParams ap = window_assemble_params(w);
+  ap.split = 4;
+  window_launch_assemble(w, ap, w->K + ap.nlinks + 1);
+  SAGE_HIP(hipGetLastError());
+  return SAGE_OK;
+}
+
 int window_linearize_set(SageWindow *w, int set, double *dst, bool local_blocks, bool merge)
 {
   if (!w || !w->finalized)
@@ -636,6 +538,16 @@
   AssembleParams ap = window_assemble_params(w);
   if (dst)
     ap.packed = dst;
+  if (w->asm_defer && !dst && !local_blocks)
+  {
+    w->asm_pending = true;
+    window_phase_mark(w, 1);
+    w->have_lin = true;
+    w->lin_epoch = set == 0 ? w->vars_epoch : 0;
+    w->spec_err_valid = false;
+    w->packed_reduced = false;
+    return SAGE_OK;
+  }
   ap.split = 4;
   int nblocks = w->K + ap.nlinks + 1;
   if (local_blocks && w->n_asm_blocks > 0)
@@ -643,10 +555,7 @@
     ap.blocks = w->asm_blocks.as<int32_t>();
     nblocks = w->n_asm_blocks;
   }
-  if (w->n_kr + w->n_km > 0)
-    hipLaunchKernelGGL(assemble_kernel<true>, dim3(nblocks * ap.split), dim3(512), 0, w->stream, ap);
-  else
-    hipLaunchKernelGGL(assemble_kernel<false>, dim3(nblocks * ap.split), dim3(512), 0, w->stream, ap);
+  window_launch_assemble(w, ap, nblocks);
   SAGE_HIP(hipGetLastError());
   window_phase_mark(w, 1);
   if (ap.packed == w->packed.as<double>())
@@ -800,6 +709,9 @@
 
 static int window_mirror_totals(SageWindow *w, bool with_err, const double *system = nullptr)
 {
+  int rcf;
+  if (!system && (rcf = window_flush_assembly(w)))
+    return rcf;
   w->mirror_epoch += 1;
   hipLaunchKernelGGL(mirror_totals_kernel, dim3(1), dim3(64), 0, w->stream,
                      (system ? system : w->packed.as<double>()) + sage_window_packed_count(w) - 4,
@@ -991,9 +903,18 @@
       return rc;
     if (w->dpt_set == 1)
       w->dpt_set = -1;
-    rc = solver_run(w->solver, w->stream, w->packed.as<double>(), w->vars[0].as<float>(), w->vars[1].as<float>(), CS,
-                    damp, c.code_prior_weight, c.scale_prior_weight, c.pose_prior_weight, w->scale_init[0],
-                    &w->pose_init[0]);
+    if (w->asm_pending)
+    {
+      w->asm_pending = false;
+      w->fused_tail_launches += 1;
+      rc = solver_run_assembling(w->solver, w->stream, window_assemble_params(w), w->n_kr + w->n_km > 0,
+                                 w->vars[0].as<float>(), w->vars[1].as<float>(), damp, c.code_prior_weight,
+                                 c.scale_prior_weight, c.pose_prior_weight, w->scale_init[0], &w->pose_init[0]);
+    }
+    else
+      rc = solver_run(w->solver, w->stream, w->packed.as<double>(), w->vars[0].as<float>(), w->vars[1].as<float>(), CS,
+                      damp, c.code_prior_weight, c.scale_prior_weight, c.pose_prior_weight, w->scale_init[0],
+                      &w->pose_init[0]);
     if (rc)
       return rc;
     window_phase_mark(w, 3);
@@ -1007,6 +928,11 @@
     return SAGE_OK;
   }
   const size_t np = sage_window_packed_count(w);
+  {
+    const int rcf = window_flush_assembly(w);
+    if (rcf)
+      return rcf;
+  }
   static const bool dbg = sage::env_flag("SAGE_DEBUG_TIMING");
   auto tnow = [] { return std::chrono::steady_clock::now(); };
   auto t_a = tnow();
@@ -1408,6 +1334,8 @@
     std::memcpy(w->h_err, ev.cur_tot, sizeof(ev.cur_tot));
 }
 
+static int window_lm_step(SageWindow *w, SageLmState *st, const SageLmConfig *cfg, LmSeq seq);
+
 extern "C" int sage_window_lm_step(SageWindow *w, SageLmState *st, const SageLmConfig *cfg)
 {
   if (!w || !st || !cfg)
@@ -1415,6 +1343,15 @@
   if (w->world > 1 && !w->allreduce)
     return SAGE_E_STATE;
   const LmSeq seq = lm_sequence_for(w, cfg);
+  w->asm_defer = seq == LmSeq::classic && w->fuse_tail && w->world == 1 && !w->allreduce && w->solver;
+  const int rc = window_lm_step(w, st, cfg, seq);
+  w->asm_defer = false;
+  const int rcf = window_flush_assembly(w);
+  return rc ? rc : rcf;
+}
+
+static int window_lm_step(SageWindow *w, SageLmState *st, const SageLmConfig *cfg, LmSeq seq)
+{
   auto clampd = [&](double d) { return std::min(std::max((double)cfg->min_damp, d), (double)cfg->max_damp); };
   if (st->iters == 0 && st->damp <= 0)
     st->damp = cfg->init_damp;
diff --git a/sage_slam_amd/csrc/window_build.hip b/sage_slam_amd/csrc/window_build.hip
--- a/sage_slam_amd/csrc/window_build.hip
+++ b/sage_slam_amd/csrc/window_build.hip
@@ -685,6 +685,7 @@
   int rc = solver_create(&w->solver, w->K, w->B, w->VS, w->links, w->stream);
   if (rc != SAGE_OK && rc != SAGE_E_UNSUPPORTED)
     return rc;
+  w->fuse_tail = w->solver && solver_can_assemble(w->solver) && !sage::env_flag("SAGE_NO_FUSED_TAIL");
   if (!fs.domain_solve)
     return SAGE_OK;
   std::vector<int32_t> lk(2 * w->links.size());
```

Measured after the change: 228,300 Mresiduals/s. -10.5%, worse.
